# spawner1145/vae-tagger

Measured on AMD Instinct MI355X. Metric: images/sec encode+tag, 1024^2 bf16, higher is better.
Workload: dtype bf16

## Files before the change

### vae_tagger_amd/csrc/attn_qk.hip

```cpp
#include <hip/hip_runtime.h>

#include <type_traits>

#include "vt_common.h"
#include "vt_kernels.h"

namespace {

constexpr int QB = 256;
constexpr int KT = 64;
constexpr int D = 512;
constexpr int KROWB = D * 2;
constexpr int KBUF = KT * KROWB;

template <int MODE>
__global__ __launch_bounds__(512, 2) void attn_qk_kernel(const AttnQkArgs a) {
    extern __shared__ __attribute__((aligned(16))) char smem[];
    if (a.gate && *a.gate != a.gate_expect) return;
    const int lane = threadIdx.x & 63;
    const int wave = __builtin_amdgcn_readfirstlane(threadIdx.x >> 6);
    const int fr = lane & 15, fq = lane >> 4;
    const int qtiles = (a.S + QB - 1) / QB;
    const int nsplit = a.nsplit > 1 ? a.nsplit : 1;
    const int logical = vt_xcd_remap(blockIdx.x, gridDim.x);
    const int per_img = qtiles * nsplit;
    const int b = logical / per_img, qs = logical - b * per_img;
    const int qt = qs / nsplit, ksp = qs - qt * nsplit;
    const bf16_t* qb = a.q + (long long)b * a.qk_bs;
    constexpr bool LIN = MODE == 4 || MODE == 5;
    const bf16_t* kb = a.k + (long long)b * (LIN ? a.k_bs : a.qk_bs);
    const int nkeys = LIN ? a.nk : a.S;
    const int ldk = LIN ? a.ldk : a.ldq;
    const int row0 = qt * QB + wave * 32;

    bf16x8 qf[2][16];
#pragma unroll
    for (int j = 0; j < 2; ++j) {
        const int row = row0 + j * 16 + fr;
        const bf16_t* src = row < a.S ? qb + (long long)row * a.ldq + fq * 8 : (const bf16_t*)a.zeros;
        const int step = row < a.S ? 32 : 0;
#pragma unroll
        for (int ks = 0; ks < 16; ++ks) qf[j][ks] = *(const bf16x8*)(src + ks * step);
    }
    float rv[2];
    float sh2[2];
#pragma unroll
    for (int j = 0; j < 2; ++j) {
        const int row = row0 + j * 16 + fr;
        rv[j] = MODE == 1 ? -__builtin_inff() : 0.f;
        if (LIN) sh2[j] = (a.qbias && row < a.S) ? a.qbias[row] : 0.f;
        else sh2[j] = (MODE >= 2 && row < a.S) ? a.rowin[(long long)b * a.row_bs + row] * 1.44269504f : 0.f;
    }
    const float alpha2 = a.alpha * 1.44269504f;

    auto stage = [&](int kt, int buf) __attribute__((always_inline)) {
#pragma unroll
        for (int jj = 0; jj < 8; ++jj) {
            const int R = wave * 8 + jj;
            const int key = kt * KT + 32 * ((R >> 5) & 1) + 8 * ((R >> 2) & 3) + 4 * ((R >> 4) & 1) + (R & 3);
            const void* src = key < nkeys ? (const void*)(kb + (long long)key * ldk + ((lane ^ (R & 15)) << 3)) : a.zeros;
            __builtin_amdgcn_global_load_lds(VT_GLOBAL_PTR(src), VT_LDS_PTR(smem + buf * KBUF + R * KROWB), 16, 0, 0);
        }
    };
    int kbase[4];
#pragma unroll
    for (int m = 0; m < 4; ++m) kbase[m] = fr * KROWB + (((((m ^ (fr >> 2)) & 3) << 2) | ((fq ^ fr) & 3)) << 4);

    f32x4 acc[4][2];
    const f32x4 zero4 = {0.f, 0.f, 0.f, 0.f};

    bf16x8 hold[2][2];
    const int sr = lane >> 2, sp = lane & 3;
    const int perm_addr = (sp * 16 + sr) << 2;
    auto store_held = [&](int kt_prev) __attribute__((always_inline)) {
        if constexpr (MODE == 5) return;
        if constexpr (MODE == 3) {
            if (row0 < a.S) {
                bf16_t* dst = a.P + (long long)b * a.p_bs + (long long)(row0 >> 5) * vt_attn_pt_slab_stride(a.S) + (long long)kt_prev * 2048 + lane * 8;
#pragma unroll
                for (int j = 0; j < 2; ++j)
#pragma unroll
#ifdef PFRAG_PLAIN
                    for (int h = 0; h < 2; ++h) *(bf16x8*)(dst + (j * 2 + h) * 512) = hold[j][h];
#else
                    for (int h = 0; h < 2; ++h) __builtin_nontemporal_store(hold[j][h], (bf16x8*)(dst + (j * 2 + h) * 512));
#endif
            }
            return;
        }
        const int key0 = kt_prev * KT + 8 * sp;
        const bool full = kt_prev * KT + KT <= nkeys;
        if constexpr (MODE == 4) {
#pragma unroll
            for (int j = 0; j < 2; ++j) {
                const int row = row0 + j * 16 + sr;
                if (row < a.S) {
                    bf16_t* dst = a.P + (long long)b * a.p_bs + (long long)row * a.ldp + key0;
                    if (full || key0 < a.ldp) *(bf16x8*)dst = hold[j][0];
                    if (full || key0 + 32 < a.ldp) *(bf16x8*)(dst + 32) = hold[j][1];
                }
            }
            return;
        }
#pragma unroll
        for (int j = 0; j < 2; ++j) {
            const int row = row0 + j * 16 + sr;
            if (row < a.S) {
                bf16_t* dst = a.P + (long long)b * a.p_bs + (long long)row * a.ldp + key0;
                if (full || key0 < a.ldp) __builtin_nontemporal_store(hold[j][0], (bf16x8*)dst);
                if (full || key0 + 32 < a.ldp) __builtin_nontemporal_store(hold[j][1], (bf16x8*)(dst + 32));
            }
        }
    };
    auto epilogue_t = [&](int kt, auto full_tag) __attribute__((always_inline)) {
        constexpr bool FULL = decltype(full_tag)::value;
        const int key0 = kt * KT + 8 * fq;
        if constexpr (MODE == 5) {
            typedef _Float16 f16x8 __attribute__((ext_vector_type(8)));
            const int nrows = a.S - row0 < 0 ? 0 : (a.S - row0 > 32 ? 32 : a.S - row0);
            const long long ob = (long long)b * a.p_bs;
#pragma unroll
            for (int h = 0; h < 2; ++h) {
                const int kk = key0 + 32 * h;
                const bool kreal = FULL || kk + 7 < nkeys;
                f32x4 b0 = {0.f, 0.f, 0.f, 0.f}, b1 = b0;
                if (a.kbias && kreal) { b0 = *(const f32x4*)(a.kbias + kk); b1 = *(const f32x4*)(a.kbias + kk + 4); }
                float v[2][8];
#pragma unroll
                for (int j = 0; j < 2; ++j) {
                    const int row = row0 + j * 16 + fr;
                    const bool ok = row < a.S && kreal;
                    const long long o = ob + (long long)row * a.ldp + kk;
                    float rs[8] = {0.f, 0.f, 0.f, 0.f, 0.f, 0.f, 0.f, 0.f};
                    if (ok && a.res_f16) {
                        const f16x8 rh = *(const f16x8*)(a.res_f16 + o);
#pragma unroll
                        for (int e = 0; e < 8; ++e) rs[e] = (float)rh[e];
                    } else if (ok && a.res_f32) {
                        const f32x4 r0 = *(const f32x4*)(a.res_f32 + o), r1 = *(const f32x4*)(a.res_f32 + o + 4);
#pragma unroll
                        for (int e = 0; e < 4; ++e) { rs[e] = r0[e]; rs[4 + e] = r1[e]; }
                    }
#pragma unroll
                    for (int e = 0; e < 8; ++e)
                        v[j][e] = fmaf(acc[2 * h + (e >> 2)][j][e & 3], a.alpha, (e < 4 ? b0[e & 3] : b1[e & 3]) + sh2[j]) + rs[e];
                    if (ok && a.out_f16) {
                        f16x8 oh;
#pragma unroll
                        for (int e = 0; e < 8; ++e) oh[e] = (f16_t)v[j][e];
                        *(f16x8*)(a.out_f16 + o) = oh;
                    } else if (ok && a.out_f32) {
                        *(f32x4*)(a.out_f32 + o) = f32x4{v[j][0], v[j][1], v[j][2], v[j][3]};
                        *(f32x4*)(a.out_f32 + o + 4) = f32x4{v[j][4], v[j][5], v[j][6], v[j][7]};
                    }
                }
                if (a.gn_partial && kreal) {
                    const float piv = __shfl(v[0][0], lane & 32, 64);
                    float s1 = 0.f, s2 = 0.f;
#pragma unroll
                    for (int j = 0; j < 2; ++j) {
                        if (row0 + j * 16 + fr < a.S) {
#pragma unroll
                            for (int e = 0; e < 8; ++e) { const float d = v[j][e] - piv; s1 += d; s2 = fmaf(d, d, s2); }
                        }
                    }
                    s1 = vt_row16_sum(s1); s2 = vt_row16_sum(s2);
                    s1 += __shfl_xor(s1, 16, 64); s2 += __shfl_xor(s2, 16, 64);
                    if (fr == 0 && (fq & 1) == 0) {
                        const float n = (float)nrows * 16.f;
                        const float ms = n > 0.f ? s1 / n : 0.f;
                        float* d = a.gn_partial + (((long long)b * a.gn_parts + (row0 >> 5)) * (nkeys >> 4) + (kk >> 4)) * 3;
                        d[0] = n; d[1] = n > 0.f ? piv + ms : 0.f; d[2] = n > 0.f ? fmaxf(s2 - s1 * ms, 0.f) : 0.f;
                    }
                }
            }
            return;
        }
#pragma unroll
        for (int j = 0; j < 2; ++j) {
#pragma unroll
            for (int i = 0; i < 4; ++i)
#pragma unroll
                for (int r = 0; r < 4; ++r) {
                    const bool real = FULL || key0 + 32 * (i >> 1) + 4 * (i & 1) + r < nkeys;
                    if (MODE == 1) {
                        if (real) rv[j] = fmaxf(rv[j], acc[i][j][r] * a.alpha);
                    } else if (MODE == 4) {
                        const int kk = key0 + 32 * (i >> 1) + 4 * (i & 1) + r;
                        const float kbv = (a.kbias && real) ? a.kbias[kk] : 0.f;
                        hold[j][i >> 1][(i & 1) * 4 + r] = (bf16_t)(real ? fmaf(acc[i][j][r], a.alpha, kbv + sh2[j]) : 0.f);
                    } else {
                        float e = __builtin_amdgcn_exp2f(fmaf(acc[i][j][r], alpha2, -sh2[j]));
                        if (!real) e = 0.f;
                        rv[j] += e;
                        hold[j][i >> 1][(i & 1) * 4 + r] = (bf16_t)e;
                    }
                }
        }
        if (MODE == 2 || MODE == 4) {
            typedef int i32x4 __attribute__((ext_vector_type(4)));
#pragma unroll
            for (int j = 0; j < 2; ++j)
#pragma unroll
                for (int h = 0; h < 2; ++h) {
                    i32x4 v = __builtin_bit_cast(i32x4, hold[j][h]);
#pragma unroll
                    for (int d = 0; d < 4; ++d) v[d] = __builtin_amdgcn_ds_bpermute(perm_addr, v[d]);
                    hold[j][h] = __builtin_bit_cast(bf16x8, v);
                }
        }
    };
    const int nkt_all = (nkeys + KT - 1) / KT;
    const int segb[5] = {0, nkt_all / 4, nkt_all / 2, (int)(3LL * nkt_all / 4), nkt_all};
    auto write_segment = [&](int seg, bool zero) __attribute__((always_inline)) {
#pragma unroll
        for (int j = 0; j < 2; ++j) {
            float v = zero ? 0.f : rv[j];
            v += __shfl_xor(v, 16);
            v += __shfl_xor(v, 32);
            const int row = row0 + j * 16 + fr;
            if (fq == 0 && row < a.S) a.rowout[(long long)seg * a.split_stride + (long long)b * a.row_bs + row] = v;
            rv[j] = 0.f;
        }
    };
    auto epilogue = [&](int kt) __attribute__((always_inline)) {
        if (kt * KT + KT <= nkeys) epilogue_t(kt, std::true_type{});
        else epilogue_t(kt, std::false_type{});
        if (MODE == 3) {
#pragma unroll
            for (int seg = 0; seg < 4; ++seg)
                if (kt + 1 == segb[seg + 1] && segb[seg + 1] > segb[seg]) write_segment(seg, false);
        }
    };

    const bool late = (wave & 4) != 0;
    const int seg0 = ksp * (4 / nsplit), seg1 = (ksp + 1) * (4 / nsplit);
    const int kt0 = MODE == 3 ? segb[seg0] : LIN ? (int)((long long)ksp * nkt_all / nsplit) : 0;
    const int nkt = MODE == 3 ? segb[seg1] : LIN ? (int)((long long)(ksp + 1) * nkt_all / nsplit) : nkt_all;
    const bool counted = MODE == 3 && row0 < a.S;
    stage(kt0, kt0 & 1);
    for (int kt = kt0; kt < nkt; ++kt) {
        if (counted && kt - kt0 > (late ? 1 : 0)) asm volatile("s_waitcnt vmcnt(4)" ::: "memory");
        else asm volatile("s_waitcnt vmcnt(0)" ::: "memory");
        __builtin_amdgcn_s_barrier();
        asm volatile("" ::: "memory");
        if (late) {
            if (kt + 1 < nkt) stage(kt + 1, (kt + 1) & 1);
            if (kt > kt0) { epilogue(kt - 1); if (MODE >= 2) store_held(kt - 1); }
        }
        const char* ks_base = smem + (kt & 1) * KBUF;
        constexpr int AHEAD = 6;
        bf16x8 kf[8];
        auto frag = [&](int idx) __attribute__((always_inline)) {
            const int ks = idx >> 2, i = idx & 3;
            return *(const bf16x8*)(ks_base + kbase[ks & 3] + (ks >> 2) * 256 + i * 16 * KROWB);
        };
#pragma unroll
        for (int p = 0; p < AHEAD; ++p) kf[p] = frag(p);
#pragma unroll
        for (int idx = 0; idx < 64; ++idx) {
            if (idx + AHEAD < 64) kf[(idx + AHEAD) & 7] = frag(idx + AHEAD);
            const int ks = idx >> 2, i = idx & 3;
#pragma unroll
            for (int j = 0; j < 2; ++j)
                acc[i][j] = __builtin_amdgcn_mfma_f32_16x16x32_bf16(kf[idx & 7], qf[j][ks], ks == 0 ? zero4 : acc[i][j], 0, 0, 0);
            __builtin_amdgcn_sched_barrier(0);
        }
        if (!late) {
            if (kt + 1 < nkt) stage(kt + 1, (kt + 1) & 1);
            epilogue(kt);
            if (MODE >= 2) store_held(kt);
        }
    }
    if (nkt > kt0 && late) {
        epilogue(nkt - 1);
        if (MODE >= 2) store_held(nkt - 1);
    }
    if constexpr (LIN) return;
    if (MODE == 3) {
#pragma unroll
        for (int seg = 0; seg < 4; ++seg)
            if (seg >= seg0 && seg < seg1 && segb[seg + 1] == segb[seg]) write_segment(seg, true);
        return;
    }
#pragma unroll
    for (int j = 0; j < 2; ++j) {
        float v = rv[j];
        const float o1 = __shfl_xor(v, 16);
        v = MODE == 1 ? fmaxf(v, o1) : v + o1;
        const float o2 = __shfl_xor(v, 32);
        v = MODE == 1 ? fmaxf(v, o2) : v + o2;
        const int row = row0 + j * 16 + fr;
        if (fq == 0 && row < a.S) a.rowout[(long long)b * a.row_bs + row] = MODE == 1 ? v : 1.f / v;
    }
}

}

bool vt_attn_qk_supported(int S, int C) { return C == D && S > 0; }

int vt_attn_linear_parts(int S) { return (S + QB - 1) / QB * 8; }

hipError_t vt_launch_attn_qk(const AttnQkArgs& a, hipStream_t s) {
    if (a.mode == 5) {
        if (!a.q || !a.k || !a.zeros || a.batch <= 0 || !vt_attn_qk_supported(a.S, a.C) || a.nk <= 0 || (a.nk % 16) || a.gate) return hipErrorInvalidValue;
        if ((a.out_f16 != nullptr) == (a.out_f32 != nullptr) || (a.res_f16 && a.res_f32)) return hipErrorInvalidValue;
        if ((a.ldq % 8) || (a.ldk % 8) || (a.qk_bs % 8) || (a.k_bs % 8) || (a.ldp % 8) || (a.p_bs % 8) || a.ldp < a.nk) return hipErrorInvalidValue;
        if ((long long)a.S * a.ldq >= (1LL << 31) || (long long)a.nk * a.ldk >= (1LL << 31)) return hipErrorInvalidValue;
        if (a.gn_partial && a.gn_parts != vt_attn_linear_parts(a.S)) return hipErrorInvalidValue;
        const int nsp = a.nsplit > 1 ? a.nsplit : 1;
        if (nsp > (a.nk + KT - 1) / KT) return hipErrorInvalidValue;
        const long long nblk5 = (long long)((a.S + QB - 1) / QB) * a.batch * nsp;
        if (nblk5 > 0x7fffffffLL) return hipErrorInvalidValue;
        static std::atomic<unsigned long long> attr5{0};
        hipError_t e5 = vt_once_per_device(attr5, [&] { return hipFuncSetAttribute((const void*)attn_qk_kernel<5>, hipFuncAttributeMaxDynamicSharedMemorySize, 2 * KBUF); });
        if (e5 != hipSuccess) return e5;
        hipLaunchKernelGGL(attn_qk_kernel<5>, dim3((unsigned)nblk5), dim3(512), 2 * KBUF, s, a);
        return hipGetLastError();
    }
    if (a.mode == 4) {
        if (!a.q || !a.k || !a.P || !a.zeros || a.batch <= 0 || !vt_attn_qk_supported(a.S, a.C) || a.nk <= 0 || a.gate) return hipErrorInvalidValue;
        if ((a.ldq % 8) || (a.ldk % 8) || (a.qk_bs % 8) || (a.k_bs % 8) || (a.ldp % 8) || (a.p_bs % 8) || a.ldp < (a.nk + 7) / 8 * 8) return hipErrorInvalidValue;
        if ((long long)a.S * a.ldq >= (1LL << 31) || (long long)a.nk * a.ldk >= (1LL << 31)) return hipErrorInvalidValue;
        const int nsp = a.nsplit > 1 ? a.nsplit : 1;
        if (nsp > (a.nk + KT - 1) / KT) return hipErrorInvalidValue;
        const long long nblk4 = (long long)((a.S + QB - 1) / QB) * a.batch * nsp;
        if (nblk4 > 0x7fffffffLL) return hipErrorInvalidValue;
        static std::atomic<unsigned long long> attr4{0};
        hipError_t e4 = vt_once_per_device(attr4, [&] { return hipFuncSetAttribute((const void*)attn_qk_kernel<4>, hipFuncAttributeMaxDynamicSharedMemorySize, 2 * KBUF); });
        if (e4 != hipSuccess) return e4;
        hipLaunchKernelGGL(attn_qk_kernel<4>, dim3((unsigned)nblk4), dim3(512), 2 * KBUF, s, a);
        return hipGetLastError();
    }
    if (!a.q || !a.k || !a.rowout || !a.zeros || a.batch <= 0 || !vt_attn_qk_supported(a.S, a.C)) return hipErrorInvalidValue;
    if (a.mode != 1 && a.mode != 2) return hipErrorInvalidValue;
    if (a.mode == 2 && (!a.P || !a.rowin || (a.p_bs % 8))) return hipErrorInvalidValue;
    if (a.mode == 2 && !a.p_frag && ((a.ldp % 8) || a.ldp < a.S)) return hipErrorInvalidValue;
    if (a.mode == 2 && a.p_frag && a.p_bs < vt_attn_pt_elems(a.S)) return hipErrorInvalidValue;
    if ((a.ldq % 8) || (a.qk_bs % 8) || a.row_bs < a.S) return hipErrorInvalidValue;
    if ((long long)a.S * a.ldq >= (1LL << 31)) return hipErrorInvalidValue;
    if (a.nsplit > 1 && (a.mode != 2 || !a.p_frag || (a.nsplit != 2 && a.nsplit != 4))) return hipErrorInvalidValue;
    if (a.mode == 2 && a.p_frag && a.split_stride < (long long)a.batch * a.row_bs) return hipErrorInvalidValue;
    const long long nblk = (long long)((a.S + QB - 1) / QB) * a.batch * (a.nsplit > 1 ? a.nsplit : 1);
    if (nblk > 0x7fffffffLL) return hipErrorInvalidValue;
    static std::atomic<unsigned long long> attr_done{0};
    hipError_t ea = vt_once_per_device(attr_done, [&] {
        hipError_t e = hipFuncSetAttribute((const void*)attn_qk_kernel<1>, hipFuncAttributeMaxDynamicSharedMemorySize, 2 * KBUF);
        if (e == hipSuccess) e = hipFuncSetAttribute((const void*)attn_qk_kernel<2>, hipFuncAttributeMaxDynamicSharedMemorySize, 2 * KBUF);
        if (e == hipSuccess) e = hipFuncSetAttribute((const void*)attn_qk_kernel<3>, hipFuncAttributeMaxDynamicSharedMemorySize, 2 * KBUF);
        return e;
    });
    if (ea != hipSuccess) return ea;
    if (a.mode == 1) hipLaunchKernelGGL(attn_qk_kernel<1>, dim3((unsigned)nblk), dim3(512), 2 * KBUF, s, a);
    else if (a.p_frag) hipLaunchKernelGGL(attn_qk_kernel<3>, dim3((unsigned)nblk), dim3(512), 2 * KBUF, s, a);
    else hipLaunchKernelGGL(attn_qk_kernel<2>, dim3((unsigned)nblk), dim3(512), 2 * KBUF, s, a);
    return hipGetLastError();
}
```

### vae_tagger_amd/csrc/conv3x3_halo.hip

```cpp
#include <type_traits>

#include "vt_common.h"
#include "vt_kernels.h"

#ifdef GNIL_DUMP
extern "C" int vt_debug_gnil_dump(float* buf) { return (int)hipMemcpyToSymbol(HIP_SYMBOL(g_gnil_dump), &buf, sizeof(buf)); }
#endif
#ifdef HALO_STAMP
__device__ unsigned long long* g_halo_stamps = nullptr;
extern "C" int vt_debug_halo_stamps(unsigned long long* buf) {
    return (int)hipMemcpyToSymbol(HIP_SYMBOL(g_halo_stamps), &buf, sizeof(buf));
}
static unsigned long long* s_stamp_ptrs[2] = {nullptr, nullptr};
static int s_stamp_H = 0, s_stamp_Cin = 0, s_stamp_nth = -1, s_stamp_seen = 0;
static bool s_stamp_on = false;
extern "C" int vt_debug_halo_stamps_nth(unsigned long long* buf, int H, int Cin, int nth) {
    s_stamp_ptrs[1] = buf; s_stamp_H = H; s_stamp_Cin = Cin; s_stamp_nth = buf ? nth : -1; s_stamp_seen = 0; s_stamp_on = false;
    return (int)hipMemcpyToSymbol(HIP_SYMBOL(g_halo_stamps), &s_stamp_ptrs[0], sizeof(void*));
}
#ifndef STAMP_TID
#define STAMP_TID 0
#endif
#define STAMP(slot)                                                                                            \
    do {                                                                                                       \
        unsigned long long t_;                                                                                 \
        __builtin_amdgcn_sched_barrier(0);                                                                     \
        asm volatile("s_memrealtime %0\n\ts_waitcnt lgkmcnt(0)" : "=s"(t_)::"memory");                         \
        __builtin_amdgcn_sched_barrier(0);                                                                     \
        if (g_halo_stamps && threadIdx.x == STAMP_TID) g_halo_stamps[(long long)blockIdx.x * 16 + (slot)] = t_; \
    } while (0)
#define STAMP_CLK(slot)                                                                                        \
    do {                                                                                                       \
        unsigned long long t_;                                                                                 \
        __builtin_amdgcn_sched_barrier(0);                                                                     \
        asm volatile("s_memtime %0\n\ts_waitcnt lgkmcnt(0)" : "=s"(t_)::"memory");                             \
        __builtin_amdgcn_sched_barrier(0);                                                                     \
        if (g_halo_stamps && threadIdx.x == STAMP_TID) g_halo_stamps[(long long)blockIdx.x * 16 + (slot)] = t_; \
    } while (0)
#else
#define STAMP(slot) do {} while (0)
#define STAMP_CLK(slot) do {} while (0)
#endif

namespace {

template <bool F16>
__device__ __forceinline__ f32x4 halo_mfma(bf16x8 a, bf16x8 b, f32x4 c) {
#ifdef HALO_F16
    constexpr bool H = true;
#else
    constexpr bool H = F16;
#endif
#ifdef GNIL_NO_MFMA
    asm volatile("" :: "v"(a), "v"(b));
    return c;
#endif
    if constexpr (H) {
        typedef _Float16 f16x8 __attribute__((ext_vector_type(8)));
        return __builtin_amdgcn_mfma_f32_16x16x32_f16(__builtin_bit_cast(f16x8, a), __builtin_bit_cast(f16x8, b), c, 0, 0, 0);
    } else {
        return __builtin_amdgcn_mfma_f32_16x16x32_bf16(a, b, c, 0, 0, 0);
    }
}

constexpr int HB = 64;
constexpr int TW = 16;
constexpr int HWID = TW + 2;
constexpr int NW_DEFAULT = 6;

__device__ __forceinline__ void wait_vmcnt(int n) {
    switch (n) {
#define C(k) case k: asm volatile("s_waitcnt vmcnt(" #k ")" ::: "memory"); break;
        C(0) C(1) C(2) C(3) C(4) C(5) C(6) C(7) C(8) C(9) C(10) C(11) C(12) C(13) C(14) C(15) C(16)
        C(17) C(18) C(19) C(20) C(21) C(22) C(23) C(24)
#undef C
        default: asm volatile("s_waitcnt vmcnt(0)" ::: "memory"); break;
    }
}

template <typename V>
__device__ __forceinline__ void wait_vmcnt_tied(int n, V& r0, V& r1) {
    switch (n) {
#define C(k) case k: asm volatile("s_waitcnt vmcnt(" #k ")" : "+v"(r0), "+v"(r1)::"memory"); break;
        C(0) C(1) C(2) C(3) C(4) C(5) C(6) C(7) C(8) C(9) C(10) C(11) C(12) C(13) C(14) C(15) C(16)
#undef C
        default: asm volatile("s_waitcnt vmcnt(0)" : "+v"(r0), "+v"(r1)::"memory"); break;
    }
}


__device__ __forceinline__ int opaque(int v) {
    asm volatile("" : "+v"(v));
    return v;
}

template <typename V>
__device__ __forceinline__ void wait_vmcnt_tied1(int n, V& r0) {
    switch (n) {
#define C(k) case k: asm volatile("s_waitcnt vmcnt(" #k ")" : "+v"(r0)::"memory"); break;
        C(0) C(1) C(2) C(3) C(4) C(5) C(6) C(7) C(8) C(9) C(10) C(11) C(12) C(13) C(14) C(15) C(16)
#undef C
        default: asm volatile("s_waitcnt vmcnt(0)" : "+v"(r0)::"memory"); break;
    }
}

template <int WP, int WC, int XT, int TPW, int NW, bool F16 = false>
__global__ __launch_bounds__(64 * WP * WC, TPW == 4 ? 4 : TPW == 16 ? 1 : 2)
void conv3x3_halo_kernel(const Conv3x3Args a) {
    static_assert(!F16 || XT == 0, "fp16 operands: plain-input tiles only");
    constexpr int NWV = WP * WC;
    constexpr int NT = 64 * NWV;
    static_assert((NWV == 8 && (TPW == 8 || (TPW == 4 && XT == 0))) || (NWV == 4 && (TPW == 8 || TPW == 16) && XT == 0),
                  "8 waves x 8 rows, 8 waves x 4 rows (two workgroups per CU), 4 waves x 8 rows (two workgroups per CU), or -- the round-4 "
                  "experiment -- 4 waves x 16 rows: ONE wave per SIMD with up to 512 registers (accumulators in AGPRs)");
    constexpr int ROWS = WP * TPW;
    constexpr int BC = WC * 64;
    constexpr int TP = TPW, TC = 4;
    constexpr int HROWS = (ROWS + 2) * HWID;
    constexpr int NLD = NWV;
    constexpr int NXW = ((HROWS + 15) / 16 + NLD - 1) / NLD;
    constexpr int XBUF = NXW * NLD * 16 * HB;
    constexpr int WPCS = BC / 16;
    constexpr int WPW = (WPCS + NLD - 1) / NLD;
    constexpr int WBUF = BC * HB;
    constexpr int LX = XT == 1 ? 2 : 1;
    constexpr int DLY = XT == 1 ? 2 : 3;
    static_assert(WPW >= 1, "BC >= 128");
    static_assert(XT == 0 || NXW + DLY <= 9, "staging must finish inside the chunk");

    extern __shared__ __attribute__((aligned(16))) char smem[];
    char* const xbase = smem;
    char* const wbase = smem + 2 * XBUF;
    float* const ssl = (float*)(wbase + NW * WBUF);

    const int lane = threadIdx.x & 63;
    const int wave = __builtin_amdgcn_readfirstlane(threadIdx.x >> 6);
    const int wp = wave / WC, wc = wave % WC;
    const bool early = wave < 4;
    const int wpw = (WPCS % NLD == 0) ? WPW : (wave < WPCS % NLD ? WPW : WPW - 1);

    STAMP(0);
    const int tiles_x = a.tiles_x, ctiles = a.ctiles, per_img = a.per_img;
    auto fdiv = [](int n, unsigned long long m, int d) -> int {
        return m ? (int)(((unsigned long long)(unsigned)n * m) >> 40) : n / d;
    };
    int logical = vt_xcd_remap(blockIdx.x, gridDim.x);
    const int b = fdiv(logical, a.m_per_img, per_img);
    logical -= b * per_img;
    const int tile = fdiv(logical, a.m_ctiles, ctiles);
    const int ct = logical - tile * ctiles;
    const int tyi = fdiv(tile, a.m_tiles_x, tiles_x);
    const int ty0 = tyi * ROWS, tx0 = (tile - tyi * tiles_x) * TW;
    const int c0 = ct * BC;

    const long long img = (long long)b * a.H * a.W * a.Cin;
    const bf16_t* Xb = a.X ? a.X + img : nullptr;
    const float* Xf = a.Xf32 ? a.Xf32 + img : nullptr;
    const int nchunk = a.Cin >> 5;
    const int nk = nchunk * 9;

    const int drow = lane >> 2;
    const int dchunk = (lane & 3) ^ (((lane >> 4) & 1) << 1);
    constexpr int NXS = XT == 0 ? 1 : NXW;
    int xsrc[NXS];
    if constexpr (XT != 0) {
#pragma unroll
        for (int j = 0; j < NXW; ++j) {
            const int hr = (j * NLD + wave) * 16 + drow;
            const int hy = hr / HWID, hx = hr - hy * HWID;
            const int iy = ty0 - 1 + hy, ix = tx0 - 1 + hx;
            const bool v = hr < HROWS && iy >= 0 && iy < a.H && ix >= 0 && ix < a.W;
            xsrc[j] = v ? (iy * a.W + ix) * a.Cin + dchunk * 8 : -1;
        }
    } else {
        xsrc[0] = 0;
    }
    const int hr0 = wave * 16 + drow;
    const int hy0 = hr0 / HWID, hx0 = hr0 - (hr0 / HWID) * HWID;
    const int wsrc0 = (c0 + wave * 16 + drow) * 32 + dchunk * 8;
    const int wstep = a.Cout * 32;

    auto issue_x_dma = [&](int chunk) {
#ifdef EXP_NO_DMA
        if (chunk >= 2) return;
#endif
        char* dst = xbase + (chunk & 1) * XBUF;
        int hy = opaque(hy0), hx = hx0, hr = hr0;
#pragma nounroll
        for (int j = 0; j < NXW; ++j) {
            const int iy = ty0 - 1 + hy, ix = tx0 - 1 + hx;
            const bool v = hr < HROWS && iy >= 0 && iy < a.H && ix >= 0 && ix < a.W;
            const void* src = v ? (const void*)(Xb + ((iy * a.W + ix) * a.Cin + dchunk * 8 + chunk * 32)) : a.zeros;
#ifndef GNIL_NO_DMA
            __builtin_amdgcn_global_load_lds(VT_GLOBAL_PTR(src), VT_LDS_PTR(dst + (j * NLD + wave) * 1024), 16, 0, 0);
#else
            asm volatile("" :: "v"(src));
#endif
            hr += NLD * 16;
            hx += (NLD * 16) % HWID; hy += (NLD * 16) / HWID;
            if (hx >= HWID) { hx -= HWID; ++hy; }
        }
    };
    constexpr bool KYMAJOR = XT == 0 && TPW == 4;
    auto issue_w = [&](int t, int tap_of_t ) {
#ifdef EXP_NO_DMA
        if (t >= NW) return;
#endif
        char* dst = wbase + (t % NW) * WBUF;
        const int src_t = KYMAJOR ? t - tap_of_t + vt_halo_step_of_tap(tap_of_t) : t;
#ifdef W_WINDOW_EXPERIMENT
        const bf16_t* wt = a.Wp + (long long)(src_t % W_WINDOW_EXPERIMENT) * wstep + opaque(wsrc0);
#else
        const bf16_t* wt = a.Wp + (long long)src_t * wstep + opaque(wsrc0);
#endif
#pragma unroll
        for (int j = 0; j < WPW; ++j)
            if (WPCS % NLD == 0 || j * NLD + wave < WPCS)
#ifndef GNIL_NO_DMA
                __builtin_amdgcn_global_load_lds(VT_GLOBAL_PTR(wt + j * NLD * 16 * 32), VT_LDS_PTR(dst + (j * NLD + wave) * 1024), 16, 0, 0);
#else
                asm volatile("" :: "v"(wt));
#endif
    };
    auto load_row = [&](int j, int chunk, f32x4& r0, f32x4& r1) {
        const int xs_j = opaque(xsrc[j]);
        const int off = xs_j >= 0 ? xs_j + chunk * 32 : 0;
        if constexpr (XT == 1) {
            const float* src = xs_j >= 0 ? Xf + off : (const float*)a.zeros;
            asm volatile("global_load_dwordx4 %0, %1, off" : "=v"(r0) : "v"(src) : "memory");
            asm volatile("global_load_dwordx4 %0, %1, off offset:16" : "=v"(r1) : "v"(src) : "memory");
        } else {
            const bf16_t* src = xs_j >= 0 ? Xb + off : (const bf16_t*)a.zeros;
            asm volatile("global_load_dwordx4 %0, %1, off" : "=v"(r0) : "v"(src) : "memory");
        }
    };
    auto write_row = [&](int j, int chunk, const f32x4& r0, const f32x4& r1) {
        const float* sp = ssl + (chunk * 32 + opaque(dchunk) * 8) * 2;
        char* dst = xbase + (chunk & 1) * XBUF + (j * NLD + wave) * 1024 + opaque(lane) * 16;
        const bool pad = xsrc[j] < 0;
#pragma unroll
        for (int hh = 0; hh < 2; ++hh) {
            float v[4];
            if constexpr (XT == 1) {
                const f32x4 r = hh ? r1 : r0;
                v[0] = r[0]; v[1] = r[1]; v[2] = r[2]; v[3] = r[3];
            } else {
                const bf16x8 h = __builtin_bit_cast(bf16x8, r0);
#pragma unroll
                for (int i = 0; i < 4; ++i) v[i] = (float)h[hh * 4 + i];
            }
            const f32x4 q0 = *(const f32x4*)(sp + hh * 8), q1 = *(const f32x4*)(sp + hh * 8 + 4);
            bf16x4 o;
            o[0] = (bf16_t)vt_silu(fmaf(v[0], q0[0], q0[1]));
            o[1] = (bf16_t)vt_silu(fmaf(v[1], q0[2], q0[3]));
            o[2] = (bf16_t)vt_silu(fmaf(v[2], q1[0], q1[1]));
            o[3] = (bf16_t)vt_silu(fmaf(v[3], q1[2], q1[3]));
            if (pad) o = bf16x4{0, 0, 0, 0};
            *(bf16x4*)(dst + hh * 8) = o;
        }
    };

    constexpr bool SPF = XT == 0;
    constexpr int LEAD = NW - 1;
    constexpr int WOUT = SPF ? LEAD - 2 : NW - 2;
    const int fr = lane & 15, fq = lane >> 4;
    f32x4 bv[4];
#pragma unroll
    for (int i = 0; i < 4; ++i)
        bv[i] = a.bias ? *(const f32x4*)(a.bias + c0 + wc * 64 + 16 * fq + 4 * i) : f32x4{0.f, 0.f, 0.f, 0.f};
    asm volatile("" ::: "memory");
    if constexpr (XT == 0) {
        issue_x_dma(0);
#pragma unroll
        for (int t = 0; t < LEAD; ++t)
            if (t < nk) issue_w(t, t % 9);
        asm volatile("" ::: "memory");
    }
    const int wfoff = (wc * 64 + fr) * HB + ((fq ^ (((fr >> 2) & 1) << 1)) << 4);
    int xsel[8];
#pragma unroll
    for (int k = 0; k < 8; ++k)
        xsel[k] = (wp * TPW * HWID + fr) * HB + ((fq ^ ((((k + fr) >> 2) & 1) << 1)) << 4);
    auto xaddr = [&](int k) -> int { return xsel[k]; };
    f32x4 acc[TC][TP];
#pragma unroll
    for (int i = 0; i < TC; ++i) {
#pragma unroll
        for (int j = 0; j < TP; ++j) acc[i][j] = bv[i];
    }

    if constexpr (XT != 0) {
        const float* ssg = a.scale_shift + (long long)b * a.Cin * 2;
        for (int i = threadIdx.x; i < a.Cin * 2; i += NT) ssl[i] = ssg[i];
        __syncthreads();
#pragma unroll
        for (int j = 0; j < NXW; ++j) {
            f32x4 r0 = {0.f, 0.f, 0.f, 0.f}, r1 = {0.f, 0.f, 0.f, 0.f};
            load_row(j, 0, r0, r1);
            if constexpr (XT == 1) wait_vmcnt_tied(0, r0, r1);
            else wait_vmcnt_tied1(0, r0);
            write_row(j, 0, r0, r1);
        }
#pragma unroll
        for (int t = 0; t < LEAD; ++t)
            if (t < nk) issue_w(t, t % 9);
    }

    constexpr bool DYR = TPW >= 8;
    bf16x8 wfc[TC], xr[DYR ? TP + 2 : TP];
    STAMP(1);
    if constexpr (SPF) {
        int ahead0 = nk - 1;
        if (ahead0 > LEAD - 1) ahead0 = LEAD - 1;
        wait_vmcnt(ahead0 * wpw);
        asm volatile("" ::: "memory");
        __builtin_amdgcn_s_barrier();
        asm volatile("" ::: "memory");
        const char* ws0 = wbase + opaque(wfoff);
#pragma unroll
        for (int i = 0; i < TC; ++i) wfc[i] = *(const bf16x8*)(ws0 + i * 16 * HB);
#pragma unroll
        for (int r = 0; r < (DYR ? TP + 2 : TP); ++r) {
            const int rel = r * HWID;
            xr[r] = *(const bf16x8*)(xbase + xaddr(rel & 7) + rel * HB);
        }
    }
    STAMP(2);
    STAMP_CLK(11);

    auto do_chunk = [&](int chunk, auto last_tag) {
        constexpr bool LAST = decltype(last_tag)::value;
        const char* xs = xbase + (chunk & 1) * XBUF;
        const int tbase = chunk * 9;
        f32x4 rq[DLY][XT == 1 ? 2 : 1];
#pragma unroll
        for (int tap = 0; tap < 9; ++tap) {
            const int t = tbase + tap;
            if constexpr (!LAST) {
                int n = WOUT * wpw;
                if (XT == 0) { if (tap >= 1 && tap <= LEAD - 1) n += NXW; }
                else { for (int r = tap - (NW - 1); r <= tap - 1; ++r) if (r >= 0 && r < NXW) n += LX; }
                wait_vmcnt(n);
            } else {
                int ahead = 8 - tap - (SPF ? 1 : 0);
                if (ahead > WOUT) ahead = WOUT;
                if (ahead < 0) ahead = 0;
                wait_vmcnt(ahead * wpw);
            }
            if (XT != 0) asm volatile("s_waitcnt lgkmcnt(0)" ::: "memory");
            asm volatile("" ::: "memory");
            __builtin_amdgcn_s_barrier();
            asm volatile("" ::: "memory");
            if constexpr (!SPF) {
                if (!LAST || tap + LEAD < 9) issue_w(t + LEAD, (tap + LEAD) % 9);
            }

            if constexpr (SPF && !DYR) {
                const bool has_next = !LAST || tap < 8;
                const int tap_n = (tap + 1) % 9;
                const int dy_n = tap_n / 3, dx_n = tap_n % 3;
                const char* xs_n = (tap == 8) ? xbase + ((chunk + 1) & 1) * XBUF : xs;
                const char* ws_n = wbase + ((t + 1) % NW) * WBUF + opaque(wfoff);
                __builtin_amdgcn_s_setprio(1);
#pragma unroll
                for (int j = 0; j < TP; ++j) {
#pragma unroll
                    for (int i = 0; i < TC; ++i)
                        acc[i][j] = halo_mfma<F16>(wfc[i], xr[j], acc[i][j]);
                    if (has_next) {
                        const int rel = (j + dy_n) * HWID + dx_n;
                        xr[j] = *(const bf16x8*)(xs_n + xaddr(rel & 7) + rel * HB);
                    }
                    if (j == TP / 2 - 1) {
                        if (!LAST || tap + LEAD < 9) issue_w(t + LEAD, (tap + LEAD) % 9);
                        if constexpr (!LAST) { if (tap == 0) issue_x_dma(chunk + 1); }
                    }
                }
                __builtin_amdgcn_s_setprio(0);
                if (has_next) {
#pragma unroll
                    for (int i = 0; i < TC; ++i) wfc[i] = *(const bf16x8*)(ws_n + i * 16 * HB);
                }
                continue;
            }
            if constexpr (SPF) {
                const int dx = tap / 3, dy = tap % 3;
                const bool has_next = !LAST || tap < 8;
                const bool next_group = !LAST || dx < 2;
                const int dx_n = (dx + 1) % 3;
                const char* xs_n = (dx == 2) ? xbase + ((chunk + 1) & 1) * XBUF : xs;
                const char* ws_n = wbase + ((t + 1) % NW) * WBUF + opaque(wfoff);
                auto refill = [&](int r) {
#ifndef EXP_NO_FRAG_READS
                    const int rel = r * HWID + dx_n;
                    xr[r] = *(const bf16x8*)(xs_n + xaddr(rel & 7) + rel * HB);
#endif
                };
                __builtin_amdgcn_s_setprio(1);
#pragma unroll
                for (int j = 0; j < TP; ++j) {
#pragma unroll
                    for (int i = 0; i < TC; ++i)
                        acc[i][j] = halo_mfma<F16>(wfc[i], xr[j + dy], acc[i][j]);
                    if (next_group) {
                        if (dy == 0 && j == 0) refill(0);
                        if (dy == 1 && j == 0) refill(1);
                        if (dy == 2) refill(j + 2);
                    }
                    if (j == TP / 2 - 1) {
                        if (!LAST || tap + LEAD < 9) issue_w(t + LEAD, (tap + LEAD) % 9);
                        if constexpr (!LAST) { if (tap == 0) issue_x_dma(chunk + 1); }
                    }
                }
                __builtin_amdgcn_s_setprio(0);
#ifndef EXP_NO_FRAG_READS
                if (has_next) {
#pragma unroll
                    for (int i = 0; i < TC; ++i) wfc[i] = *(const bf16x8*)(ws_n + i * 16 * HB);
                }
#endif
                continue;
            }
            const char* ws = wbase + (t % NW) * WBUF + opaque(wfoff);
            const int dx = tap / 3, dy = tap % 3;
            bf16x8 wf[TC];
#pragma unroll
            for (int i = 0; i < TC; ++i) wf[i] = *(const bf16x8*)(ws + i * 16 * HB);

            constexpr bool STAGE = !LAST && XT != 0;
            const int r = tap - DLY;
            auto stage_row = [&]() {
                int n = DLY * wpw;
                for (int q = r + 1; q < tap; ++q) if (q < NXW) n += LX;
                if constexpr (XT == 1) wait_vmcnt_tied(n, rq[r % DLY][0], rq[r % DLY][1]);
                else wait_vmcnt_tied1(n, rq[r % DLY][0]);
                write_row(r, chunk + 1, rq[r % DLY][0], rq[r % DLY][XT == 1 ? 1 : 0]);
            };
            if constexpr (STAGE) {
                if (r >= 0 && r < NXW) {
                    if (early) stage_row();
                    __builtin_amdgcn_sched_barrier(0);
                }
            }
            __builtin_amdgcn_s_setprio(1);
#pragma unroll
            for (int jh = 0; jh < TP; jh += 4) {
                bf16x8 xf[4];
#pragma unroll
                for (int j = 0; j < 4; ++j) {
                    const int rel = (jh + j + dy) * HWID + dx;
                    xf[j] = *(const bf16x8*)(xs + xaddr(rel & 7) + rel * HB);
                }
#pragma unroll
                for (int j = 0; j < 4; ++j)
#pragma unroll
                    for (int i = 0; i < TC; ++i)
                        acc[i][jh + j] = halo_mfma<F16>(wf[i], xf[j], acc[i][jh + j]);
            }
            __builtin_amdgcn_s_setprio(0);
            if constexpr (STAGE) {
                if (r >= 0 && r < NXW) {
                    __builtin_amdgcn_sched_barrier(0);
                    if (!early) stage_row();
                }
                if (tap < NXW) load_row(tap, chunk + 1, rq[tap % DLY][0], rq[tap % DLY][XT == 1 ? 1 : 0]);
            }
        }
    };
    for (int chunk = 0; chunk + 1 < nchunk; ++chunk) do_chunk(chunk, std::false_type{});
    do_chunk(nchunk - 1, std::true_type{});
    if constexpr (XT == 0 && TPW >= 8) {
        if (a.scX) {
            const bf16_t* Xs = a.scX + (long long)b * a.H * a.W * a.scCin;
            const int scn = a.scCin >> 5;
#pragma nounroll
            for (int c = 0; c < scn; ++c) {
                asm volatile("s_waitcnt lgkmcnt(0)" ::: "memory");
                __builtin_amdgcn_s_barrier();
                asm volatile("" ::: "memory");
                {
                    int hy = opaque(hy0), hx = hx0, hr = hr0;
#pragma nounroll
                    for (int j = 0; j < NXW; ++j) {
                        const int iy = ty0 - 1 + hy, ix = tx0 - 1 + hx;
                        const bool v = hr < HROWS && iy >= 0 && iy < a.H && ix >= 0 && ix < a.W;
                        const void* src = v ? (const void*)(Xs + ((iy * a.W + ix) * a.scCin + dchunk * 8 + c * 32)) : a.zeros;
                        __builtin_amdgcn_global_load_lds(VT_GLOBAL_PTR(src), VT_LDS_PTR(xbase + (j * NLD + wave) * 1024), 16, 0, 0);
                        hr += NLD * 16;
                        hx += (NLD * 16) % HWID; hy += (NLD * 16) / HWID;
                        if (hx >= HWID) { hx -= HWID; ++hy; }
                    }
                    const bf16_t* wt = a.scW + (long long)c * wstep + opaque(wsrc0);
#pragma unroll
                    for (int j = 0; j < WPW; ++j)
                        if (WPCS % NLD == 0 || j * NLD + wave < WPCS)
                            __builtin_amdgcn_global_load_lds(VT_GLOBAL_PTR(wt + j * NLD * 16 * 32), VT_LDS_PTR(wbase + (j * NLD + wave) * 1024), 16, 0, 0);
                }
                wait_vmcnt(0);
                asm volatile("" ::: "memory");
                __builtin_amdgcn_s_barrier();
                asm volatile("" ::: "memory");
                const char* ws = wbase + opaque(wfoff);
                bf16x8 wf[TC];
#pragma unroll
                for (int i = 0; i < TC; ++i) wf[i] = *(const bf16x8*)(ws + i * 16 * HB);
#pragma unroll
                for (int jh = 0; jh < TP; jh += 4) {
                    bf16x8 xf[4];
#pragma unroll
                    for (int j = 0; j < 4; ++j) {
                        const int rel = (jh + j + 1) * HWID + 1;
                        xf[j] = *(const bf16x8*)(xbase + xaddr(rel & 7) + rel * HB);
                    }
#pragma unroll
                    for (int j = 0; j < 4; ++j)
#pragma unroll
                        for (int i = 0; i < TC; ++i)
                            acc[i][jh + j] = halo_mfma<F16>(wf[i], xf[j], acc[i][jh + j]);
                }
            }
        }
    }
    STAMP_CLK(12);
    STAMP(3);
#ifdef HALO_STAMP
    asm volatile("s_nop 0" :: "v"(acc[0][0]), "v"(acc[TC - 1][TP - 1]));
    STAMP(8);
#endif

    const int HWp = a.H * a.W;
    const long long ob = (long long)b * HWp * a.Cout;
    const int x = tx0 + fr;
    const int cw = c0 + wc * 64 + 16 * fq;
    constexpr int RPCS = TPW * 2;
    constexpr bool RES_DMA = NWV * RPCS * 1024 <= 2 * XBUF + NW * WBUF;
    char* const rbuf = smem + wave * (RPCS * 1024);
    if (RES_DMA && a.res_f16) {
        asm volatile("s_waitcnt lgkmcnt(0)" ::: "memory");
        __syncthreads();
#pragma unroll 4
        for (int pc = 0; pc < RPCS; ++pc) {
            const int pp = pc * 8 + (lane >> 3);
            const int yy = ty0 + wp * TPW + (pp >> 4), xx = tx0 + (pp & 15);
            const int lc = (lane & 7) ^ (pp & 7);
            const void* src = (yy < a.H && xx < a.W)
                ? (const void*)(a.res_f16 + ob + ((long long)yy * a.W + xx) * a.Cout + c0 + wc * 64 + lc * 8) : a.zeros;
            __builtin_amdgcn_global_load_lds(VT_GLOBAL_PTR(src), VT_LDS_PTR(rbuf + pc * 1024), 16, 0, 0);
        }
        asm volatile("s_waitcnt vmcnt(0)" ::: "memory");
    }
    unsigned valid = 0;
#pragma unroll
    for (int j = 0; j < TP; ++j) {
        const int y = ty0 + wp * TPW + j;
        if (y >= a.H || x >= a.W) continue;
        valid |= 1u << j;
        const long long o = ob + ((long long)y * a.W + x) * a.Cout + cw;
#pragma unroll
        for (int i = 0; i < TC; ++i) {
            f32x4 v = acc[i][j];
            if (a.res) v += *(const f32x4*)(a.res + o + 4 * i);
            if (a.out_f32) *(f32x4*)(a.out_f32 + o + 4 * i) = v;
            acc[i][j] = v;
        }
        if (a.res_f16) {
            const int pp = j * 16 + fr;
#pragma unroll
            for (int i = 0; i < TC; i += 2) {
                typedef _Float16 f16x8 __attribute__((ext_vector_type(8)));
                const f16x8 rh = RES_DMA ? *(const f16x8*)(rbuf + pp * 128 + (((2 * fq + (i >> 1)) ^ (pp & 7)) << 4))
                                         : *(const f16x8*)(a.res_f16 + o + 4 * i);
#pragma unroll
                for (int r = 0; r < 4; ++r) { acc[i][j][r] += (float)rh[r]; acc[i + 1][j][r] += (float)rh[4 + r]; }
            }
        }
        if (a.out_f16) {
#pragma unroll
            for (int i = 0; i < TC; i += 2) {
                typedef _Float16 f16x8 __attribute__((ext_vector_type(8)));
                f16x8 h;
#pragma unroll
                for (int r = 0; r < 4; ++r) { h[r] = (f16_t)acc[i][j][r]; h[4 + r] = (f16_t)acc[i + 1][j][r]; }
                *(f16x8*)(a.out_f16 + o + 4 * i) = h;
            }
        }
        if (a.out_bf16) {
            const long long o16 = a.out16_planar ? (((long long)(b * (a.Cout >> 5) + (cw >> 5)) * a.H + y) * a.W + x) * 32 + (cw & 31) : o;
#pragma unroll
            for (int i = 0; i < TC; i += 2) {
                if (a.out16_f16) {
                    typedef _Float16 f16x8o __attribute__((ext_vector_type(8)));
                    f16x8o h;
#pragma unroll
                    for (int r = 0; r < 4; ++r) { h[r] = (f16_t)acc[i][j][r]; h[4 + r] = (f16_t)acc[i + 1][j][r]; }
                    *(f16x8o*)((f16_t*)a.out_bf16 + o16 + 4 * i) = h;
                } else {
                bf16x8 h;
#pragma unroll
                for (int r = 0; r < 4; ++r) { h[r] = (bf16_t)acc[i][j][r]; h[4 + r] = (bf16_t)acc[i + 1][j][r]; }
#ifdef EPI_NOSTORE
                asm volatile("" :: "v"(h));
#else
                *(bf16x8*)(a.out_bf16 + o16 + 4 * i) = h;
#endif
                }
            }
        }
    }
    STAMP(4);
    if (a.gn_partial) {
        __syncthreads();
        STAMP(10);
        const int G = a.Cout / a.gn_cpg;
        float* out = a.gn_partial + (((long long)b * a.ptiles + tile) * G + c0 / a.gn_cpg) * 3;
        vt_gn_epilogue_partials_il<TC, TP>(acc, valid, a.gn_cpg, wp, WP, wc * 64, BC, (float*)smem, out);
    }
#ifdef HALO_STAMP
    STAMP(5);
    asm volatile("s_waitcnt vmcnt(0)" ::: "memory");
    STAMP(6);
    if (g_halo_stamps && threadIdx.x == STAMP_TID) {
        unsigned hw, xcc;
        asm volatile("s_getreg_b32 %0, hwreg(HW_REG_HW_ID)" : "=s"(hw));
        asm volatile("s_getreg_b32 %0, hwreg(HW_REG_XCC_ID)" : "=s"(xcc));
        g_halo_stamps[(long long)blockIdx.x * 16 + 7] = ((unsigned long long)xcc << 32) | hw;
    }
#endif
}

template <int WP, int WC, int XT, int TPW, int NW = NW_DEFAULT, bool F16 = false>
hipError_t launch(const Conv3x3Args& a, hipStream_t s) {
    constexpr int ROWS = WP * TPW, BC = WC * 64, NWV = WP * WC;
    constexpr int HROWS = (ROWS + 2) * HWID;
    constexpr int NXW = ((HROWS + 15) / 16 + NWV - 1) / NWV;
    const int smem = 2 * NXW * NWV * 16 * HB + NW * BC * HB + (XT ? a.Cin * 8 : 0);
    if (smem > 160 * 1024) return hipErrorInvalidValue;
    static std::atomic<unsigned long long> attr_done{0};
    auto kern = conv3x3_halo_kernel<WP, WC, XT, TPW, NW, F16>;
    hipError_t ea = vt_once_per_device(attr_done, [&] { return hipFuncSetAttribute((const void*)kern, hipFuncAttributeMaxDynamicSharedMemorySize, 160 * 1024); });
    if (ea != hipSuccess) return ea;
    const long long tiles = (long long)((a.W + TW - 1) / TW) * ((a.H + ROWS - 1) / ROWS);
    const long long nblk = tiles * (a.Cout / BC) * a.batch;
    if (nblk <= 0 || nblk > 0x7fffffffLL) return hipErrorInvalidValue;
    Conv3x3Args k = a;
    k.tiles_x = (a.W + TW - 1) / TW; k.ctiles = a.Cout / BC; k.per_img = (int)(tiles * k.ctiles); k.ptiles = (int)tiles;
    auto magic = [&](long long d) -> unsigned long long {
        return (nblk * d < (1LL << 40) && nblk < (1LL << 23)) ? ((1ULL << 40) / (unsigned long long)d + 1ULL) : 0ULL;
    };
    k.m_per_img = magic(k.per_img); k.m_ctiles = magic(k.ctiles); k.m_tiles_x = magic(k.tiles_x);
#ifdef HALO_STAMP
    if (s_stamp_nth >= 0) {
        const bool on = a.H == s_stamp_H && a.Cin == s_stamp_Cin && s_stamp_seen++ == s_stamp_nth;
        if (on != s_stamp_on) {
            (void)hipMemcpyToSymbolAsync(HIP_SYMBOL(g_halo_stamps), &s_stamp_ptrs[on ? 1 : 0], sizeof(void*), 0, hipMemcpyHostToDevice, s);
            s_stamp_on = on;
        }
    }
#endif
#ifdef GNIL_ONE_WG
    hipLaunchKernelGGL(kern, dim3((unsigned)nblk), dim3(64 * NWV), smem > 90 * 1024 ? smem : 90 * 1024, s, k);
#else
    hipLaunchKernelGGL(kern, dim3((unsigned)nblk), dim3(64 * NWV), smem, s, k);
#endif
    return hipGetLastError();
}

__global__ void repack_ohwi_kernel(const bf16_t* __restrict__ w, bf16_t* __restrict__ wp, int Cin, int Cout) {
    const long long n = (long long)Cout * 9 * Cin;
    const long long i = (long long)blockIdx.x * blockDim.x + threadIdx.x;
    if (i >= n) return;
    const int ci = (int)(i % Cin);
    const int tap = (int)((i / Cin) % 9);
    const int co = (int)(i / ((long long)Cin * 9));
    const int row = (co & ~63) + vt_halo_row_of_cout(co & 63);
    wp[(((long long)(ci >> 5) * 9 + vt_halo_step_of_tap(tap)) * Cout + row) * 32 + (ci & 31)] = w[i];
}

}

hipError_t vt_launch_repack_ohwi_to_halo(const bf16_t* w, bf16_t* wp, int Cin, int Cout, hipStream_t s) {
    const long long n = (long long)Cout * 9 * Cin;
    hipLaunchKernelGGL(repack_ohwi_kernel, dim3((unsigned)((n + 255) / 256)), dim3(256), 0, s, w, wp, Cin, Cout);
    return hipGetLastError();
}

namespace {
enum HaloVariant { HV_2208_4 = 0, HV_4204_4, HV_4208_6, HV_2408_6, HV_XT1_128, HV_XT1_256, HV_XT2_128, HV_XT2_256, HV_2216_6 };
HaloVariant halo_variant(int Cout, int xt, int occ2, bool has_sc) {
    const bool big = (Cout % 256) == 0;
    if (xt == 1) return big ? HV_XT1_256 : HV_XT1_128;
    if (xt == 2) return big ? HV_XT2_256 : HV_XT2_128;
    if (occ2 == 4) return HV_2216_6;
    if (occ2 == 3 || (occ2 == 2 && !big)) return HV_2208_4;
    if (occ2 && !big && !has_sc) return HV_4204_4;
    return big ? HV_2408_6 : HV_4208_6;
}
int halo_variant_rows(HaloVariant v) {
    switch (v) {
        case HV_4208_6: case HV_XT1_128: case HV_XT2_128: case HV_2216_6: return 32;
        default: return 16;
    }
}
}

int vt_conv3x3_halo_tiles(int H, int W, int Cout, int xt, int occ2, int has_sc) {
    const int rows = halo_variant_rows(halo_variant(Cout, xt, occ2, has_sc != 0));
    return ((W + TW - 1) / TW) * ((H + rows - 1) / rows);
}
int vt_conv3x3_halo_tiles_max(int H, int W) { return ((W + TW - 1) / TW) * ((H + 15) / 16); }

bool vt_conv3x3_halo_supported(int Cin, int Cout) { return Cin >= 32 && (Cin % 32) == 0 && (Cout % 128) == 0; }
bool vt_conv3x3_halo_f16_supported(int Cout, int occ2, int has_sc) { return halo_variant(Cout, 0, occ2, has_sc != 0) == HV_2208_4; }

static int halo_xt(const Conv3x3Args& a) { return a.scale_shift ? (a.Xf32 ? 1 : 2) : 0; }

int vt_conv3x3_halo_config(const Conv3x3Args& a) {
    switch (halo_variant(a.Cout, halo_xt(a), a.occ2, a.scX != nullptr)) {
        case HV_2208_4: return 3;
        case HV_4204_4: return 4;
        case HV_4208_6: return 5;
        case HV_2408_6: return 6;
        case HV_2216_6: return 5;
        case HV_XT1_128: case HV_XT1_256: return 7;
        default: return 8;
    }
}

hipError_t vt_launch_conv3x3_halo(const Conv3x3Args& a, hipStream_t s) {
    if (!a.Wp || !a.zeros || (!a.out_f32 && !a.out_bf16 && !a.out_f16)) return hipErrorInvalidValue;
    if ((a.res && a.res_f16) || (a.res_f16 && a.out_f32)) return hipErrorInvalidValue;
    if (!vt_conv3x3_halo_supported(a.Cin, a.Cout) || a.batch <= 0 || a.H <= 0 || a.W <= 0) return hipErrorInvalidValue;
    if (a.gn_partial && a.gn_cpg != 4 && a.gn_cpg != 8 && a.gn_cpg != 16) return hipErrorInvalidValue;
    if ((long long)a.H * a.W * a.Cin >= (1LL << 31)) return hipErrorInvalidValue;
    if ((a.scX != nullptr) != (a.scW != nullptr)) return hipErrorInvalidValue;
    if (a.scX && (a.scCin <= 0 || (a.scCin % 32) || a.scale_shift || (long long)a.H * a.W * a.scCin >= (1LL << 31))) return hipErrorInvalidValue;
    if ((long long)(a.Cin / 32) * 9 * a.Cout * 32 >= (1LL << 31)) return hipErrorInvalidValue;
    if (a.occ2 < 0 || a.occ2 > 4) return hipErrorInvalidValue;
    const int xt = halo_xt(a);
    if (xt == 1 ? (a.X != nullptr) : (a.X == nullptr || a.Xf32 != nullptr)) return hipErrorInvalidValue;
    if (a.f16 && (xt != 0 || halo_variant(a.Cout, xt, a.occ2, a.scX != nullptr) != HV_2208_4)) return hipErrorInvalidValue;
    if (a.f16) return launch<2, 2, 0, 8, 4, true>(a, s);
    switch (halo_variant(a.Cout, xt, a.occ2, a.scX != nullptr)) {
        case HV_2208_4: return launch<2, 2, 0, 8, 4>(a, s);
        case HV_4204_4: return launch<4, 2, 0, 4, 4>(a, s);
        case HV_4208_6: return launch<4, 2, 0, 8>(a, s);
        case HV_2408_6: return launch<2, 4, 0, 8>(a, s);
        case HV_2216_6: return launch<2, 2, 0, 16, 6>(a, s);
        case HV_XT1_128: return launch<4, 2, 1, 8>(a, s);
        case HV_XT1_256: return launch<2, 4, 1, 8>(a, s);
        case HV_XT2_128: return launch<4, 2, 2, 8>(a, s);
        default: return launch<2, 4, 2, 8>(a, s);
    }
}
```

### vae_tagger_amd/csrc/conv3x3_s2_halo.hip

```cpp
#include <type_traits>

#include "vt_common.h"
#include "vt_kernels.h"

namespace {

constexpr int HB = 64;
constexpr int TW = 16, ROWS = 16;
constexpr int WP = 2, WC = 2, TP = 8, TC = 4;
constexpr int NWV = WP * WC, NT = 64 * NWV, BC = WC * 64;
constexpr int NW = 3, LEAD = NW - 1;
constexpr int WBUF = BC * HB;
constexpr int WPW = BC / 16 / NWV;
constexpr int NXB = 3;
#ifndef S2_W_AT
#define S2_W_AT (TP / 2 - 1)
#endif
constexpr int XSTRIDE = 289 * HB;
constexpr int SMEM = NXB * XSTRIDE + NW * WBUF;
static_assert(2 * SMEM <= 160 * 1024, "two workgroups per CU");

__host__ __device__ constexpr int pl_py(int pl) { return pl >> 1; }
__host__ __device__ constexpr int pl_px(int pl) { return pl & 1; }
__host__ __device__ constexpr int pl_pitch(int pl) { return pl_px(pl) ? 16 : 17; }
__host__ __device__ constexpr int pl_hrows(int pl) { return pl_py(pl) ? 16 : 17; }
__host__ __device__ constexpr int pl_rows(int pl) { return pl_pitch(pl) * pl_hrows(pl); }
__host__ __device__ constexpr int pl_pieces(int pl) { return pl_rows(pl) / 16; }
__host__ __device__ constexpr int nx_pl(int pl) { return pl == 3 ? 4 : 5; }
__host__ __device__ constexpr int st_plane(int p) { return p < 4 ? 0 : p < 6 ? 1 : p < 8 ? 2 : 3; }
__host__ __device__ constexpr int st_dx(int p) { return (p == 2 || p == 3 || p == 7) ? 1 : 0; }
__host__ __device__ constexpr int st_dy(int p) { return (p == 1 || p == 3 || p == 5) ? 1 : 0; }
__host__ __device__ constexpr bool st_two(int p) { return p < 6; }
__host__ __device__ constexpr int ng_plane(int p) { return p < 2 ? 0 : p < 4 ? 1 : p < 7 ? 2 : p < 8 ? 3 : 0; }
__host__ __device__ constexpr int ng_dx(int p) { return (p < 2 || p == 6) ? 1 : 0; }
__host__ __device__ constexpr int ng_rows(int p) { return (p < 4 || p == 8) ? 9 : 8; }

__device__ __forceinline__ void wait_vmcnt(int n) {
    switch (n) {
#define C(k) case k: asm volatile("s_waitcnt vmcnt(" #k ")" ::: "memory"); break;
        C(0) C(1) C(2) C(3) C(4) C(5) C(6) C(7) C(8) C(9) C(10) C(11) C(12)
#undef C
        default: asm volatile("s_waitcnt vmcnt(0)" ::: "memory"); break;
    }
}
__device__ __forceinline__ int opaque(int v) {
    asm volatile("" : "+v"(v));
    return v;
}
__device__ __forceinline__ int opaque_s(int v) {
    asm volatile("" : "+s"(v));
    return v;
}

template <bool F16>
__global__ __launch_bounds__(NT, 2) void conv3x3_s2_halo_kernel(const Conv3x3S2Args a) {
    extern __shared__ __attribute__((aligned(16))) char smem[];
    char* const xbase = smem;
    char* const wbase = smem + NXB * XSTRIDE;
    const int lane = threadIdx.x & 63;
    const int wave = __builtin_amdgcn_readfirstlane(threadIdx.x >> 6);
    const int wp = wave / WC, wc = wave % WC;
    const int fr = lane & 15, fq = lane >> 4;

    auto fdiv = [](int n, unsigned long long m, int d) -> int {
        return m ? (int)(((unsigned long long)(unsigned)n * m) >> 40) : n / d;
    };
    int logical = vt_xcd_remap(blockIdx.x, gridDim.x);
    const int b = fdiv(logical, a.m_per_img, a.per_img);
    logical -= b * a.per_img;
    const int tile = fdiv(logical, a.m_ctiles, a.ctiles);
    const int ct = logical - tile * a.ctiles;
    const int tyi = fdiv(tile, a.m_tiles_x, a.tiles_x);
    const int ty0 = tyi * ROWS, tx0 = (tile - tyi * a.tiles_x) * TW;
    const int c0 = ct * BC;
    const bf16_t* Xb = a.X + (long long)b * a.H * a.W * a.Cin;
    const int xpix = a.x_planar ? 32 : a.Cin, xchunk = a.x_planar ? a.H * a.W * 32 : 32;
    const int nchunk = a.Cin >> 5;
    const int nk = nchunk * 9;

    const int drow = lane >> 2;
    const int dchunk = (lane & 3) ^ (((lane >> 4) & 1) << 1);
    const int wsrc0 = (c0 + wave * 16 + drow) * 32 + dchunk * 8;
    const int wstep = a.Cout * 32;

    auto issue_x = [&](auto pl_tag, int chunk, int slot) {
        constexpr int PL = decltype(pl_tag)::value;
        constexpr int PITCH = pl_pitch(PL), PY = pl_py(PL), PX = pl_px(PL), NP = pl_pieces(PL), NXP = nx_pl(PL);
        constexpr int NPT = PL == 0 ? NP + 1 : NP;
        char* dst = xbase + slot * XSTRIDE;
#pragma nounroll
        for (int j = 0; j < NXP; ++j) {
            int piece = j * NWV + wave;
            if (piece >= NPT) piece = NPT - 1;
            const int row0 = (PL == 0 && piece == NP) ? pl_rows(0) - 16 : piece * 16;
            const int hr = row0 + opaque(drow);
            const int hy = hr / PITCH, hx = hr - hy * PITCH;
            const int iy = 2 * (ty0 + hy) + PY, ix = 2 * (tx0 + hx) + PX;
            const int lch = (lane & 3) ^ (((hr >> 2) & 1) << 1);
            const void* src = (iy < a.H && ix < a.W) ? (const void*)(Xb + ((iy * a.W + ix) * xpix + chunk * xchunk + lch * 8)) : a.zeros;
            __builtin_amdgcn_global_load_lds(VT_GLOBAL_PTR(src), VT_LDS_PTR(dst + row0 * HB), 16, 0, 0);
        }
    };
    auto issue_w = [&](int t) {
        char* dst = wbase + (t % NW) * WBUF;
        const bf16_t* wt = a.Wp + (long long)t * wstep + opaque(wsrc0);
#pragma unroll
        for (int j = 0; j < WPW; ++j)
            __builtin_amdgcn_global_load_lds(VT_GLOBAL_PTR(wt + j * NWV * 16 * 32), VT_LDS_PTR(dst + (j * NWV + wave) * 1024), 16, 0, 0);
    };

    issue_x(std::integral_constant<int, 0>{}, 0, 0);
    issue_w(0);
    issue_w(1);
    issue_x(std::integral_constant<int, 1>{}, 0, 1);
    asm volatile("" ::: "memory");

    const int wfoff = (wc * 64 + fr) * HB + ((fq ^ (((fr >> 2) & 1) << 1)) << 4);
    int xsel[8];
#pragma unroll
    for (int k = 0; k < 8; ++k) xsel[k] = fr * HB + ((fq ^ ((((k + fr) >> 2) & 1) << 1)) << 4);
    const int wpoff17 = wp * TP * 17 * HB, wpoff16 = wp * TP * 16 * HB;
    auto xfrag = [&](const char* buf , int pitch , int r, int dx) -> bf16x8 {
        const int rel = r * pitch + dx;
        return *(const bf16x8*)(buf + xsel[rel & 7] + rel * HB);
    };
    auto xfrag_after = [&](const char* buf, int pitch, int r, int dx, const f32x4& after) -> bf16x8 {
        const int rel = r * pitch + dx;
        int off = xsel[rel & 7];
        asm volatile("" : "+v"(off) : "v"(after));
        return *(const bf16x8*)(buf + off + rel * HB);
    };

    f32x4 acc[TC][TP];
#pragma unroll
    for (int i = 0; i < TC; ++i)
#pragma unroll
        for (int j = 0; j < TP; ++j) acc[i][j] = f32x4{0.f, 0.f, 0.f, 0.f};

    bf16x8 wfc[TC], xr[TP + 1];
    {
        wait_vmcnt(WPW + nx_pl(1));
        asm volatile("" ::: "memory");
        __builtin_amdgcn_s_barrier();
        asm volatile("" ::: "memory");
        const char* ws0 = wbase + opaque(wfoff);
#pragma unroll
        for (int i = 0; i < TC; ++i) wfc[i] = *(const bf16x8*)(ws0 + i * 16 * HB);
#pragma unroll
        for (int r = 0; r < TP + 1; ++r) xr[r] = xfrag(xbase + opaque_s(wpoff17), 17, r, 0);
    }

    int cm = 0;
    auto slot_of = [&](int cmod, int pl) -> int { const int s = cmod + pl; return s >= 3 ? (s >= 6 ? s - 6 : s - 3) : s; };

    auto do_chunk = [&](int chunk, auto last_tag) {
        constexpr bool LAST = decltype(last_tag)::value;
        const int tbase = chunk * 9;
        const int cmn = cm == 2 ? 0 : cm + 1;
#pragma unroll
        for (int p = 0; p < 9; ++p) {
            const int t = tbase + p;
            {
                int n = 0;
                if (p == 1) n = nx_pl(2);
                if (p == 4) n = nx_pl(3);
                if (p == 6 && !LAST) n = nx_pl(0);
                if (p == 0) n = nx_pl(1);
                wait_vmcnt(n);
            }
            asm volatile("" ::: "memory");
            __builtin_amdgcn_s_barrier();
            asm volatile("" ::: "memory");
            constexpr int dummy = 0; (void)dummy;
            const int pl = st_plane(p), dy = st_dy(p);
            const bool two = st_two(p);
            const bool has_next = !LAST || p < 8;
            const int npl = ng_plane(p), ndx = ng_dx(p), nrows = ng_rows(p);
            const int npitch = pl_pitch(npl);
            const bool next_chunk = p == 8;
            const char* xs_n = xbase + opaque_s(slot_of(next_chunk ? cmn : cm, npl) * XSTRIDE + (npitch == 17 ? wpoff17 : wpoff16));
            const char* ws_n = wbase + ((t + 1) % NW) * WBUF + opaque(wfoff);
            (void)pl;
            auto refill = [&](int r, const f32x4& after) {
                if (has_next && r < nrows) xr[r] = xfrag_after(xs_n, npitch, r, ndx, after);
            };
            __builtin_amdgcn_s_setprio(1);
#pragma unroll
            for (int j = 0; j < TP; ++j) {
#pragma unroll
                for (int i = 0; i < TC; ++i)
                    if constexpr (F16) {
                        typedef _Float16 f16x8m __attribute__((ext_vector_type(8)));
                        acc[i][j] = __builtin_amdgcn_mfma_f32_16x16x32_f16(__builtin_bit_cast(f16x8m, wfc[i]), __builtin_bit_cast(f16x8m, xr[two ? j + dy : j]), acc[i][j], 0, 0, 0);
                    } else {
                        acc[i][j] = __builtin_amdgcn_mfma_f32_16x16x32_bf16(wfc[i], xr[two ? j + dy : j], acc[i][j], 0, 0, 0);
                    }
                if (two) {
                    if (dy == 0) { if (j == 0) refill(0, acc[TC - 1][j]); }
                    else refill(j + 1, acc[TC - 1][j]);
                } else {
                    refill(j, acc[TC - 1][j]);
                    if (j == TP - 1) refill(TP, acc[TC - 1][j]);
                }
                if (j == S2_W_AT) {
                    if (!LAST || p + LEAD < 9) issue_w(t + LEAD);
                }
                if (j == TP / 2 - 1) {
                    if (p == 0) issue_x(std::integral_constant<int, 2>{}, chunk, slot_of(cm, 2));
                    if (p == 3) issue_x(std::integral_constant<int, 3>{}, chunk, slot_of(cm, 3));
                    if constexpr (!LAST) {
                        if (p == 5) issue_x(std::integral_constant<int, 0>{}, chunk + 1, slot_of(cmn, 0));
                        if (p == 8) issue_x(std::integral_constant<int, 1>{}, chunk + 1, slot_of(cmn, 1));
                    }
                }
            }
            __builtin_amdgcn_s_setprio(0);
            if (has_next) {
#pragma unroll
                for (int i = 0; i < TC; ++i) wfc[i] = *(const bf16x8*)(ws_n + i * 16 * HB);
            }
            __builtin_amdgcn_sched_barrier(0);
        }
        cm = cmn;
    };
    for (int chunk = 0; chunk + 1 < nchunk; ++chunk) do_chunk(chunk, std::false_type{});
    do_chunk(nchunk - 1, std::true_type{});
    (void)nk;
#pragma unroll
    for (int i = 0; i < TC; ++i)
#pragma unroll
        for (int j = 0; j < TP; ++j) asm volatile("" : "+v"(acc[i][j]));
    asm volatile("" ::: "memory");

    const long long ob = (long long)b * a.Ho * a.Wo * a.Cout;
    const int x = tx0 + fr;
    const int cw = c0 + wc * 64 + 16 * fq;
    f32x4 bv[4];
#pragma unroll
    for (int i = 0; i < 4; ++i) bv[i] = a.bias ? *(const f32x4*)(a.bias + cw + 4 * i) : f32x4{0.f, 0.f, 0.f, 0.f};
    unsigned valid = 0;
#pragma unroll
    for (int j = 0; j < TP; ++j) {
        const int y = ty0 + wp * TP + j;
        if (y >= a.Ho || x >= a.Wo) continue;
        valid |= 1u << j;
        const long long o = ob + ((long long)y * a.Wo + x) * a.Cout + cw;
#pragma unroll
        for (int i = 0; i < TC; ++i) {
            f32x4 v = acc[i][j] + bv[i];
            if (a.res) v += *(const f32x4*)(a.res + o + 4 * i);
            if (a.out_f32) *(f32x4*)(a.out_f32 + o + 4 * i) = v;
            acc[i][j] = v;
        }
        typedef _Float16 f16x8 __attribute__((ext_vector_type(8)));
        if (a.out_f16) {
#pragma unroll
            for (int i = 0; i < TC; i += 2) {
                f16x8 h;
#pragma unroll
                for (int r = 0; r < 4; ++r) { h[r] = (f16_t)acc[i][j][r]; h[4 + r] = (f16_t)acc[i + 1][j][r]; }
                *(f16x8*)(a.out_f16 + o + 4 * i) = h;
            }
        }
        if (a.out_bf16) {
#pragma unroll
            for (int i = 0; i < TC; i += 2) {
                if (a.out16_f16) {
                    f16x8 h;
#pragma unroll
                    for (int r = 0; r < 4; ++r) { h[r] = (f16_t)acc[i][j][r]; h[4 + r] = (f16_t)acc[i + 1][j][r]; }
                    *(f16x8*)((f16_t*)a.out_bf16 + o + 4 * i) = h;
                } else {
                    bf16x8 h;
#pragma unroll
                    for (int r = 0; r < 4; ++r) { h[r] = (bf16_t)acc[i][j][r]; h[4 + r] = (bf16_t)acc[i + 1][j][r]; }
                    *(bf16x8*)(a.out_bf16 + o + 4 * i) = h;
                }
            }
        }
    }
    if (a.gn_partial) {
        asm volatile("s_waitcnt lgkmcnt(0)" ::: "memory");
        __syncthreads();
        const int G = a.Cout / a.gn_cpg;
        float* out = a.gn_partial + (((long long)b * a.ptiles + tile) * G + c0 / a.gn_cpg) * 3;
        vt_gn_epilogue_partials_il<TC, TP>(acc, valid, a.gn_cpg, wp, WP, wc * 64, BC, (float*)smem, out);
    }
}

__global__ void repack_ohwi_s2_kernel(const bf16_t* __restrict__ w, bf16_t* __restrict__ wp, int Cin, int Cout) {
    const long long n = (long long)Cout * 9 * Cin;
    const long long i = (long long)blockIdx.x * blockDim.x + threadIdx.x;
    if (i >= n) return;
    const int ci = (int)(i % Cin);
    const int tap = (int)((i / Cin) % 9);
    const int co = (int)(i / ((long long)Cin * 9));
    const int row = (co & ~63) + vt_halo_row_of_cout(co & 63);
    wp[(((long long)(ci >> 5) * 9 + vt_s2_step_of_tap(tap)) * Cout + row) * 32 + (ci & 31)] = w[i];
}

}

bool vt_conv3x3_s2_supported(int Cin, int Cout) { return Cin >= 32 && (Cin % 32) == 0 && (Cout % 128) == 0; }
int vt_conv3x3_s2_tiles(int Ho, int Wo) { return ((Wo + TW - 1) / TW) * ((Ho + ROWS - 1) / ROWS); }

hipError_t vt_launch_repack_ohwi_to_s2(const bf16_t* w, bf16_t* wp, int Cin, int Cout, hipStream_t s) {
    const long long n = (long long)Cout * 9 * Cin;
    hipLaunchKernelGGL(repack_ohwi_s2_kernel, dim3((unsigned)((n + 255) / 256)), dim3(256), 0, s, w, wp, Cin, Cout);
    return hipGetLastError();
}

hipError_t vt_launch_conv3x3_s2(const Conv3x3S2Args& a, hipStream_t s) {
    if (!a.X || !a.Wp || !a.zeros || (!a.out_f32 && !a.out_bf16 && !a.out_f16)) return hipErrorInvalidValue;
    if (!vt_conv3x3_s2_supported(a.Cin, a.Cout) || a.batch <= 0 || a.H < 2 || a.W < 2) return hipErrorInvalidValue;
    if (a.gn_partial && a.gn_cpg != 4 && a.gn_cpg != 8 && a.gn_cpg != 16) return hipErrorInvalidValue;
    if ((long long)a.H * a.W * a.Cin >= (1LL << 31)) return hipErrorInvalidValue;
    if ((long long)(a.Cin / 32) * 9 * a.Cout * 32 >= (1LL << 31)) return hipErrorInvalidValue;
    static std::atomic<unsigned long long> attr_done{0};
    hipError_t ea = vt_once_per_device(attr_done, [&] {
        hipError_t e = hipFuncSetAttribute((const void*)conv3x3_s2_halo_kernel<false>, hipFuncAttributeMaxDynamicSharedMemorySize, SMEM);
        if (e == hipSuccess) e = hipFuncSetAttribute((const void*)conv3x3_s2_halo_kernel<true>, hipFuncAttributeMaxDynamicSharedMemorySize, SMEM);
        return e;
    });
    if (ea != hipSuccess) return ea;
    Conv3x3S2Args k = a;
    k.Ho = a.H / 2; k.Wo = a.W / 2;
    const long long tiles = vt_conv3x3_s2_tiles(k.Ho, k.Wo);
    const long long nblk = tiles * (a.Cout / BC) * a.batch;
    if (nblk <= 0 || nblk > 0x7fffffffLL) return hipErrorInvalidValue;
    k.tiles_x = (k.Wo + TW - 1) / TW; k.ctiles = a.Cout / BC; k.per_img = (int)(tiles * k.ctiles); k.ptiles = (int)tiles;
    auto magic = [&](long long d) -> unsigned long long {
        return (nblk * d < (1LL << 40) && nblk < (1LL << 23)) ? ((1ULL << 40) / (unsigned long long)d + 1ULL) : 0ULL;
    };
    k.m_per_img = magic(k.per_img); k.m_ctiles = magic(k.ctiles); k.m_tiles_x = magic(k.tiles_x);
    if (a.f16) hipLaunchKernelGGL(conv3x3_s2_halo_kernel<true>, dim3((unsigned)nblk), dim3(NT), SMEM, s, k);
    else hipLaunchKernelGGL(conv3x3_s2_halo_kernel<false>, dim3((unsigned)nblk), dim3(NT), SMEM, s, k);
    return hipGetLastError();
}
```

### vae_tagger_amd/csrc/conv3x3_up2.hip

```cpp
#include "vt_common.h"
#include "vt_kernels.h"

namespace {

constexpr int HB = 64;
constexpr int TW = 16;
constexpr int HWID = TW + 2;
constexpr int ROWS = 8;
constexpr int NWV = 4;
constexpr int TPW = 2;
constexpr int BC = 64;
constexpr int TC = 4;
constexpr int HROWS = (ROWS + 2) * HWID;
constexpr int XPCS = (HROWS + 15) / 16;
constexpr int XBUF = XPCS * 16 * HB;
constexpr int WBLK = BC * HB;
constexpr int WPCS = 16 * BC / 16;
constexpr int SMEM = XBUF + 16 * WBLK;

template <bool F16>
__device__ __forceinline__ f32x4 up2_mfma(bf16x8 a, bf16x8 b, f32x4 c) {
    if constexpr (F16) {
        typedef _Float16 f16x8 __attribute__((ext_vector_type(8)));
        return __builtin_amdgcn_mfma_f32_16x16x32_f16(__builtin_bit_cast(f16x8, a), __builtin_bit_cast(f16x8, b), c, 0, 0, 0);
    } else {
        return __builtin_amdgcn_mfma_f32_16x16x32_bf16(a, b, c, 0, 0, 0);
    }
}

template <bool F16>
__global__ __launch_bounds__(64 * NWV, 2)
void conv3x3_up2_kernel(const ConvUp2Args a) {
    extern __shared__ __attribute__((aligned(16))) char smem[];
    char* const xbase = smem;
    char* const wbase = smem + XBUF;

    const int lane = threadIdx.x & 63;
    const int wave = __builtin_amdgcn_readfirstlane(threadIdx.x >> 6);
    const int fr = lane & 15, fq = lane >> 4;

    int logical = vt_xcd_remap(blockIdx.x, gridDim.x);
    const int per_img = a.ptiles * a.ctiles;
    const int b = logical / per_img;
    logical -= b * per_img;
    const int tile = logical / a.ctiles;
    const int ct = logical - tile * a.ctiles;
    const int tyi = tile / a.tiles_x;
    const int ty0 = tyi * ROWS, tx0 = (tile - tyi * a.tiles_x) * TW;
    const int c0 = ct * BC;

    const bf16_t* Xb = a.X + (long long)b * a.H * a.W * a.Cin;
    const int nchunk = a.Cin >> 5;

    const int drow = lane >> 2;
    const int dchunk = (lane & 3) ^ (((lane >> 4) & 1) << 1);
    auto stage = [&](int chunk) {
#pragma nounroll
        for (int pc = wave; pc < XPCS; pc += NWV) {
            const int hr = pc * 16 + drow;
            const int hy = hr / HWID, hx = hr - hy * HWID;
            const int iy = ty0 - 1 + hy, ix = tx0 - 1 + hx;
            const bool v = hr < HROWS && iy >= 0 && iy < a.H && ix >= 0 && ix < a.W;
            const void* src = v ? (const void*)(Xb + ((iy * a.W + ix) * a.Cin + dchunk * 8 + chunk * 32)) : a.zeros;
            __builtin_amdgcn_global_load_lds(VT_GLOBAL_PTR(src), VT_LDS_PTR(xbase + pc * 1024), 16, 0, 0);
        }
        const bf16_t* wsrc = a.Wp + ((long long)chunk * 16 * a.Cout + c0 + drow) * 32 + dchunk * 8;
#pragma nounroll
        for (int pc = wave; pc < WPCS; pc += NWV) {
            const int q = pc >> 2, part = pc & 3;
            __builtin_amdgcn_global_load_lds(VT_GLOBAL_PTR(wsrc + ((long long)q * a.Cout + part * 16) * 32), VT_LDS_PTR(wbase + pc * 1024), 16, 0, 0);
        }
    };

    f32x4 acc[TC][8];
#pragma unroll
    for (int i = 0; i < TC; ++i) {
        const f32x4 bv = a.bias ? *(const f32x4*)(a.bias + c0 + 16 * fq + 4 * i) : f32x4{0.f, 0.f, 0.f, 0.f};
#pragma unroll
        for (int j = 0; j < 8; ++j) acc[i][j] = bv;
    }

    const int wfoff = fr * HB + ((fq ^ (((fr >> 2) & 1) << 1)) << 4);

#pragma nounroll
    for (int chunk = 0; chunk < nchunk; ++chunk) {
        __syncthreads();
        stage(chunk);
        asm volatile("s_waitcnt vmcnt(0)" ::: "memory");
        __syncthreads();
        bf16x8 xf[4][3];
#pragma unroll
        for (int r = 0; r < 4; ++r) {
#pragma unroll
            for (int s = 0; s < 3; ++s) {
                const int row = (wave * TPW + r) * HWID + s + fr;
                xf[r][s] = *(const bf16x8*)(xbase + row * HB + ((fq ^ (((row >> 2) & 1) << 1)) << 4));
            }
        }
#pragma unroll
        for (int p = 0; p < 4; ++p) {
            const int pa = p >> 1, pb = p & 1;
#pragma unroll
            for (int t = 0; t < 4; ++t) {
                const int ry = t >> 1, rx = t & 1;
                const char* ws = wbase + (p * 4 + t) * WBLK + wfoff;
                bf16x8 wf[TC];
#pragma unroll
                for (int i = 0; i < TC; ++i) wf[i] = *(const bf16x8*)(ws + i * 16 * HB);
#pragma unroll
                for (int j = 0; j < TPW; ++j) {
#pragma unroll
                    for (int i = 0; i < TC; ++i)
                        acc[i][p * 2 + j] = up2_mfma<F16>(wf[i], xf[j + ry + pa][rx + pb], acc[i][p * 2 + j]);
                }
            }
        }
    }

    const int Ho = 2 * a.H, Wo = 2 * a.W;
    const long long ob = (long long)b * Ho * Wo * a.Cout;
    const int lx = tx0 + fr;
    const int cw = c0 + 16 * fq;
    unsigned valid = 0;
#pragma unroll
    for (int p = 0; p < 4; ++p) {
#pragma unroll
        for (int j = 0; j < TPW; ++j) {
            const int ly = ty0 + wave * TPW + j;
            if (ly >= a.H || lx >= a.W) continue;
            const int jj = p * 2 + j;
            valid |= 1u << jj;
            const long long o = ob + ((long long)(2 * ly + (p >> 1)) * Wo + (2 * lx + (p & 1))) * a.Cout + cw;
            if (a.out_f32) {
#pragma unroll
                for (int i = 0; i < TC; ++i) *(f32x4*)(a.out_f32 + o + 4 * i) = acc[i][jj];
            }
            typedef _Float16 f16x8 __attribute__((ext_vector_type(8)));
            if (a.out_f16) {
#pragma unroll
                for (int i = 0; i < TC; i += 2) {
                    f16x8 h;
#pragma unroll
                    for (int r = 0; r < 4; ++r) { h[r] = (f16_t)acc[i][jj][r]; h[4 + r] = (f16_t)acc[i + 1][jj][r]; }
                    *(f16x8*)(a.out_f16 + o + 4 * i) = h;
                }
            }
            if (a.out_16) {
#pragma unroll
                for (int i = 0; i < TC; i += 2) {
                    if (a.out16_f16) {
                        f16x8 h;
#pragma unroll
                        for (int r = 0; r < 4; ++r) { h[r] = (f16_t)acc[i][jj][r]; h[4 + r] = (f16_t)acc[i + 1][jj][r]; }
                        *(f16x8*)((f16_t*)a.out_16 + o + 4 * i) = h;
                    } else {
                        bf16x8 h;
#pragma unroll
                        for (int r = 0; r < 4; ++r) { h[r] = (bf16_t)acc[i][jj][r]; h[4 + r] = (bf16_t)acc[i + 1][jj][r]; }
                        *(bf16x8*)(a.out_16 + o + 4 * i) = h;
                    }
                }
            }
        }
    }
    if (a.gn_partial) {
        __syncthreads();
        const int G = a.Cout / a.gn_cpg;
        float* out = a.gn_partial + (((long long)b * a.ptiles + tile) * G + c0 / a.gn_cpg) * 3;
        vt_gn_epilogue_partials_il<TC, 8>(acc, valid, a.gn_cpg, wave, NWV, 0, BC, (float*)smem, out);
    }
}

template <bool F16>
hipError_t launch_up2(const ConvUp2Args& a, hipStream_t s) {
    static std::atomic<unsigned long long> attr_done{0};
    auto kern = conv3x3_up2_kernel<F16>;
    hipError_t ea = vt_once_per_device(attr_done, [&] { return hipFuncSetAttribute((const void*)kern, hipFuncAttributeMaxDynamicSharedMemorySize, SMEM); });
    if (ea != hipSuccess) return ea;
    ConvUp2Args k = a;
    k.tiles_x = (a.W + TW - 1) / TW;
    k.ptiles = k.tiles_x * ((a.H + ROWS - 1) / ROWS);
    k.ctiles = a.Cout / BC;
    const long long nblk = (long long)k.ptiles * k.ctiles * a.batch;
    if (nblk <= 0 || nblk > 0x7fffffffLL) return hipErrorInvalidValue;
    hipLaunchKernelGGL(kern, dim3((unsigned)nblk), dim3(64 * NWV), SMEM, s, k);
    return hipGetLastError();
}

__global__ void pack_up2_kernel(const float* __restrict__ w, bf16_t* __restrict__ wp_bf16, f16_t* __restrict__ wp_f16, int Cin, int Cout) {
    const long long n = (long long)Cout * Cin * 16;
    const long long idx = (long long)blockIdx.x * blockDim.x + threadIdx.x;
    if (idx >= n) return;
    const int q = (int)(idx & 15);
    const int ci = (int)((idx >> 4) % Cin);
    const int co = (int)((idx >> 4) / Cin);
    const int pa = q >> 3, pb = (q >> 2) & 1, ry = (q >> 1) & 1, rx = q & 1;
    const int ky0 = pa == 0 ? (ry == 0 ? 0 : 1) : (ry == 0 ? 0 : 2), ky1 = pa == 0 ? (ry == 0 ? 0 : 2) : (ry == 0 ? 1 : 2);
    const int kx0 = pb == 0 ? (rx == 0 ? 0 : 1) : (rx == 0 ? 0 : 2), kx1 = pb == 0 ? (rx == 0 ? 0 : 2) : (rx == 0 ? 1 : 2);
    const float* wt = w + ((long long)co * Cin + ci) * 9;
    float sum = 0.f;
    bool first = true;
    for (int ky = ky0; ky <= ky1; ++ky)
        for (int kx = kx0; kx <= kx1; ++kx) {
            const float v = wt[ky * 3 + kx];
            sum = first ? v : __fadd_rn(sum, v);
            first = false;
        }
    const int row = (co & ~63) + vt_halo_row_of_cout(co & 63);
    const long long d = (((long long)(ci >> 5) * 16 + q) * Cout + row) * 32 + (ci & 31);
    if (wp_bf16) wp_bf16[d] = (bf16_t)sum;
    if (wp_f16) wp_f16[d] = (f16_t)sum;
}

__global__ void pack_f32_oihw_kernel(const float* __restrict__ w, bf16_t* __restrict__ dst, int Cin, int Cout, int layout, int f16) {
    const long long n = (long long)Cout * Cin * 9;
    const long long idx = (long long)blockIdx.x * blockDim.x + threadIdx.x;
    if (idx >= n) return;
    const int tap = (int)(idx % 9);
    const int ci = (int)((idx / 9) % Cin);
    const int co = (int)(idx / ((long long)Cin * 9));
    const int row = (co & ~63) + vt_halo_row_of_cout(co & 63);
    const long long d = layout == 0 ? ((long long)co * 9 + tap) * Cin + ci
                                    : (((long long)(ci >> 5) * 9 + vt_halo_step_of_tap(tap)) * Cout + row) * 32 + (ci & 31);
    if (f16) ((f16_t*)dst)[d] = (f16_t)w[idx]; else dst[d] = (bf16_t)w[idx];
}

__global__ __launch_bounds__(256)
void upsample2x_nhwc16_kernel(const uint4* __restrict__ x, uint4* __restrict__ y, int H, int W, int C8, long long n) {
    const long long idx = (long long)blockIdx.x * blockDim.x + threadIdx.x;
    if (idx >= n) return;
    const int c = (int)(idx % C8);
    long long p = idx / C8;
    const int X = (int)(p % (2 * W)); p /= 2 * W;
    const int Y = (int)(p % (2 * H));
    const long long b = p / (2 * H);
    y[idx] = x[((b * H + (Y >> 1)) * W + (X >> 1)) * C8 + c];
}

}

bool vt_conv3x3_up2_supported(int Cin, int Cout) { return Cin >= 32 && (Cin % 32) == 0 && Cout >= BC && (Cout % BC) == 0; }
int vt_conv3x3_up2_tiles(int H, int W) { return ((W + TW - 1) / TW) * ((H + ROWS - 1) / ROWS); }

hipError_t vt_launch_conv3x3_up2(const ConvUp2Args& a, hipStream_t s) {
    if (!a.X || !a.Wp || !a.zeros || (!a.out_f32 && !a.out_f16 && !a.out_16)) return hipErrorInvalidValue;
    if (!vt_conv3x3_up2_supported(a.Cin, a.Cout) || a.batch <= 0 || a.H <= 0 || a.W <= 0) return hipErrorInvalidValue;
    if (a.gn_partial && a.gn_cpg != 4 && a.gn_cpg != 8 && a.gn_cpg != 16) return hipErrorInvalidValue;
    if ((long long)a.H * a.W * a.Cin >= (1LL << 31)) return hipErrorInvalidValue;
    if ((long long)a.H * 2 + 1 >= (1LL << 30) || (long long)a.W * 2 + 1 >= (1LL << 30)) return hipErrorInvalidValue;
    return a.f16 ? launch_up2<true>(a, s) : launch_up2<false>(a, s);
}

hipError_t vt_launch_pack_up2(const float* w_oihw, bf16_t* wp_bf16, f16_t* wp_f16, int Cin, int Cout, hipStream_t s) {
    const long long n = (long long)Cout * Cin * 16;
    if (!w_oihw || (!wp_bf16 && !wp_f16) || n <= 0 || (n + 255) / 256 > 0x7fffffffLL) return hipErrorInvalidValue;
    hipLaunchKernelGGL(pack_up2_kernel, dim3((unsigned)((n + 255) / 256)), dim3(256), 0, s, w_oihw, wp_bf16, wp_f16, Cin, Cout);
    return hipGetLastError();
}

hipError_t vt_launch_pack_f32_oihw(const float* w_oihw, bf16_t* dst, int Cin, int Cout, int layout, int f16, hipStream_t s) {
    const long long n = (long long)Cout * Cin * 9;
    if (!w_oihw || !dst || n <= 0 || (n + 255) / 256 > 0x7fffffffLL || (layout == 1 && (Cin % 32 || Cout % 64))) return hipErrorInvalidValue;
    hipLaunchKernelGGL(pack_f32_oihw_kernel, dim3((unsigned)((n + 255) / 256)), dim3(256), 0, s, w_oihw, dst, Cin, Cout, layout, f16);
    return hipGetLastError();
}

hipError_t vt_launch_upsample2x_nhwc16(const void* x, void* y, int B, int H, int W, int C, hipStream_t s) {
    if (!x || !y || B <= 0 || H <= 0 || W <= 0 || C <= 0 || (C % 8)) return hipErrorInvalidValue;
    const long long n = (long long)B * 2 * H * 2 * W * (C / 8);
    if ((n + 255) / 256 > 0x7fffffffLL) return hipErrorInvalidValue;
    hipLaunchKernelGGL(upsample2x_nhwc16_kernel, dim3((unsigned)((n + 255) / 256)), dim3(256), 0, s, (const uint4*)x, (uint4*)y, H, W, C / 8, n);
    return hipGetLastError();
}
```

### vae_tagger_amd/csrc/conv_gemm.hip

```cpp
#include "vt_common.h"
#include "vt_kernels.h"

namespace {

constexpr int ROWB = 128;

template <int BP, int BC, int WP, int WC, bool F8 = false, bool F16 = false>
__device__ __forceinline__ void conv_gemm_tile(const ConvGemmArgs& a, char* smem, int logical) {
    static_assert(!(F8 && F16), "one operand type");
    static_assert(WP * WC == 8, "8 waves per workgroup");
    constexpr int ES = F8 ? 1 : 2;
    constexpr int BK = ROWB / ES;
    constexpr int CE = 16 / ES;
    constexpr int TP = BP / WP / 16;
    constexpr int TC = BC / WC / 16;
    constexpr int XI = BP / 8;
    constexpr int WI = BC / 8;
    constexpr int NXJ = (XI + 7) / 8;
    constexpr int NWJ = (WI + 7) / 8;
    constexpr int STAGE_BYTES = (BP + BC) * ROWB;

    const int lane = threadIdx.x & 63;
    const int wave = __builtin_amdgcn_readfirstlane(threadIdx.x >> 6);
    const int wp = wave / WC, wc = wave % WC;

    const int HWo = a.Hout * a.Wout;
    const int ptiles = (HWo + BP - 1) / BP;
    const int ctiles = (a.Cout + BC - 1) / BC;
    const int per_img = ptiles * ctiles;
    const int b = logical / per_img;
    logical -= b * per_img;
    const int p0 = (logical / ctiles) * BP;
    const int c0 = (logical % ctiles) * BC;

    const char* Xb = (const char*)a.X + (long long)b * a.x_bs * ES;
    const char* Wb = (const char*)a.W + (long long)b * a.w_bs * ES;

    const int lrow = lane >> 3;
    const int lchunk = (lane & 7) ^ lrow;
    const int ntaps = a.ksize * a.ksize;
    const int ncb = (a.Cin + BK - 1) / BK;
    const bool chunk_tail_possible = (a.Cin % BK) != 0;

    int xoff[NXJ];
    unsigned xmask[NXJ];
#pragma unroll
    for (int j = 0; j < NXJ; ++j) {
        const int r = (j * 8 + wave) * 8 + lrow;
        const int p = p0 + r;
        const bool rv = (r < BP) && (p < HWo);
        const int oy = p / a.Wout, ox = p - oy * a.Wout;
        const int iy0 = oy * a.stride - a.pad, ix0 = ox * a.stride - a.pad;
        xoff[j] = (iy0 * a.Win + ix0) * a.ldx + lchunk * CE;
        unsigned m = 0;
        if (rv) {
            for (int t = 0; t < ntaps; ++t) {
                const int ky = t / a.ksize, kx = t - ky * a.ksize;
                const int iy = iy0 + ky, ix = ix0 + kx;
                if (iy >= 0 && iy < a.Hin && ix >= 0 && ix < a.Win) m |= 1u << t;
            }
        }
        xmask[j] = m;
    }
    int woff[NWJ];
    bool wvalid[NWJ];
#pragma unroll
    for (int j = 0; j < NWJ; ++j) {
        const int rblk = j * 8 + wave;
        const int rl = rblk * 8 + lrow;
        const int n = c0 + (TC == 4 ? (rl & ~63) + (rl & 3) + 4 * ((rl >> 4) & 3) + 16 * ((rl >> 2) & 3) : rl);
        wvalid[j] = (rblk < WI) && (n < a.Wrows);
        woff[j] = n * a.ldw + lchunk * CE;
    }

    auto stage = [&](int tap, int cb, int buf) {
        char* xs = smem + buf * STAGE_BYTES;
        char* ws = xs + BP * ROWB;
        const int ky = (tap * 11) >> 5, kx = tap - ky * 3;
        const int doff = (a.ksize == 1) ? 0 : (ky * a.Win + kx) * a.ldx;
        const int k0 = cb * BK;
        const bool cv = !chunk_tail_possible || (k0 + lchunk * CE < a.Cin);
#pragma unroll
        for (int j = 0; j < NXJ; ++j) {
            const int rblk = j * 8 + wave;
            if (XI % 8 == 0 || rblk < XI) {
                const bool v = ((xmask[j] >> tap) & 1u) && cv;
                const void* src = v ? (const void*)(Xb + (long long)(xoff[j] + doff + k0) * ES) : a.zeros;
                if (a.x_stream) __builtin_amdgcn_global_load_lds(VT_GLOBAL_PTR(src), VT_LDS_PTR(xs + rblk * 1024), 16, 0, 2);
                else __builtin_amdgcn_global_load_lds(VT_GLOBAL_PTR(src), VT_LDS_PTR(xs + rblk * 1024), 16, 0, 0);
            }
        }
#pragma unroll
        for (int j = 0; j < NWJ; ++j) {
            const int rblk = j * 8 + wave;
            if (WI % 8 == 0 || rblk < WI) {
                const bool v = wvalid[j] && cv;
                const void* src = v ? (const void*)(Wb + (long long)(woff[j] + tap * a.Cin + k0) * ES) : a.zeros;
                __builtin_amdgcn_global_load_lds(VT_GLOBAL_PTR(src), VT_LDS_PTR(ws + rblk * 1024), 16, 0, 0);
            }
        }
    };

    const int frow = lane & 15;
    const int fq = lane >> 4;
    const int foff0 = frow * ROWB + (((0 + fq) ^ (lane & 7)) << 4);
    const int foff1 = frow * ROWB + (((4 + fq) ^ (lane & 7)) << 4);

    f32x4 acc[TC][TP];
#pragma unroll
    for (int i = 0; i < TC; ++i)
#pragma unroll
        for (int j = 0; j < TP; ++j) acc[i][j] = f32x4{0.f, 0.f, 0.f, 0.f};

    const int nk = ntaps * ncb;
    stage(0, 0, 0);
    int tap_n = 0, cb_n = 1;
    if (cb_n == ncb) { cb_n = 0; tap_n = 1; }

    for (int t = 0; t < nk; ++t) {
        __syncthreads();
        if (t + 1 < nk) {
            stage(tap_n, cb_n, (t + 1) & 1);
            if (++cb_n == ncb) { cb_n = 0; ++tap_n; }
        }
        const char* xs = smem + (t & 1) * STAGE_BYTES + (wp * (BP / WP)) * ROWB;
        const char* ws = smem + (t & 1) * STAGE_BYTES + BP * ROWB + (wc * (BC / WC)) * ROWB;
        if constexpr (F8) {
            typedef int i32x4 __attribute__((ext_vector_type(4)));
            typedef int i32x8 __attribute__((ext_vector_type(8)));
            const int fa = frow * ROWB + (((2 * fq) ^ (lane & 7)) << 4), fb = frow * ROWB + (((2 * fq + 1) ^ (lane & 7)) << 4);
            i32x8 wf[TC], xf[TP];
#pragma unroll
            for (int i = 0; i < TC; ++i) {
                const i32x4 lo = *(const i32x4*)(ws + i * 16 * ROWB + fa), hi = *(const i32x4*)(ws + i * 16 * ROWB + fb);
                wf[i] = i32x8{lo[0], lo[1], lo[2], lo[3], hi[0], hi[1], hi[2], hi[3]};
            }
#pragma unroll
            for (int j = 0; j < TP; ++j) {
                const i32x4 lo = *(const i32x4*)(xs + j * 16 * ROWB + fa), hi = *(const i32x4*)(xs + j * 16 * ROWB + fb);
                xf[j] = i32x8{lo[0], lo[1], lo[2], lo[3], hi[0], hi[1], hi[2], hi[3]};
            }
#pragma unroll
            for (int i = 0; i < TC; ++i)
#pragma unroll
                for (int j = 0; j < TP; ++j)
                    acc[i][j] = __builtin_amdgcn_mfma_scale_f32_16x16x128_f8f6f4(wf[i], xf[j], acc[i][j], 0, 0, 0, 127, 0, 127);
        } else {
#pragma unroll
            for (int kk = 0; kk < 2; ++kk) {
                const int fo = kk ? foff1 : foff0;
                bf16x8 wf[TC], xf[TP];
#pragma unroll
                for (int i = 0; i < TC; ++i) wf[i] = *(const bf16x8*)(ws + i * 16 * ROWB + fo);
#pragma unroll
                for (int j = 0; j < TP; ++j) xf[j] = *(const bf16x8*)(xs + j * 16 * ROWB + fo);
#pragma unroll
                for (int i = 0; i < TC; ++i)
#pragma unroll
                    for (int j = 0; j < TP; ++j) {
                        if constexpr (F16) {
                            typedef _Float16 f16x8m __attribute__((ext_vector_type(8)));
                            acc[i][j] = __builtin_amdgcn_mfma_f32_16x16x32_f16(__builtin_bit_cast(f16x8m, wf[i]), __builtin_bit_cast(f16x8m, xf[j]), acc[i][j], 0, 0, 0);
                        } else {
                            acc[i][j] = __builtin_amdgcn_mfma_f32_16x16x32_bf16(wf[i], xf[j], acc[i][j], 0, 0, 0);
                        }
                    }
            }
        }
    }

    const long long ob = (long long)b * a.o_bs;
    const float* resb = a.res ? a.res + (long long)b * a.r_bs : nullptr;
    const f16_t* resh = a.res_f16 ? a.res_f16 + (long long)b * a.r_bs : nullptr;
    const bool wide16 = TC == 4 && (a.ldo % 8) == 0 && (a.o_bs % 8) == 0;
    const bool staged = wide16 && a.out_mode == 0 && (a.out_bf16 || a.out_f16) && c0 + BC <= a.Cout;
    unsigned valid = 0;
    const bool nomask = c0 + BC <= a.Wrows;
#pragma unroll
    for (int j = 0; j < TP; ++j) {
        const int p = p0 + wp * (BP / WP) + j * 16 + frow;
        if (p >= HWo) continue;
        valid |= 1u << j;
        const int cg0 = c0 + wc * (BC / WC) + (TC == 4 ? fq * 16 : fq * 4);
        const float rin = a.row_in ? a.row_in[(long long)b * a.row_bs + p] : 0.f;
        float racc = a.row_mode == 1 ? -__builtin_inff() : 0.f;
        const float alpha2 = a.alpha * 1.44269504f, rin2 = rin * 1.44269504f;
#pragma unroll
        for (int i = 0; i < TC; ++i) {
            const int cg = cg0 + (TC == 4 ? i * 4 : i * 16);
            if (cg >= a.Cout) continue;
            f32x4 v = acc[i][j] * a.alpha;
            if (a.col_scale) v *= *(const f32x4*)(a.col_scale + cg);
            if (a.row_mode) {
                if (a.row_mode == 3) {
                    v *= rin;
                } else if (a.row_mode == 2) {
#pragma unroll
                    for (int r = 0; r < 4; ++r) {
                        const float e = __builtin_amdgcn_exp2f(fmaf(acc[i][j][r], alpha2, -rin2));
                        v[r] = (nomask || cg + r < a.Wrows) ? e : 0.f;
                        racc += v[r];
                    }
                } else {
#pragma unroll
                    for (int r = 0; r < 4; ++r)
                        if (cg + r < a.Wrows) racc = fmaxf(racc, v[r]);
                    continue;
                }
            }
            if (a.bias_mode == 1) {
                const f32x4 bv = *(const f32x4*)(a.bias + cg);
                v += bv;
            } else if (a.bias_mode == 2) {
                const float bv = a.bias[p];
                v += f32x4{bv, bv, bv, bv};
            }
            if (a.out_mode == 1) {
#pragma unroll
                for (int r = 0; r < 4; ++r)
                    if (cg + r < a.cout_keep)
                        a.out_f32[ob + (long long)(cg + r) * HWo + p] = v[r] * a.post_scale + a.post_shift;
                continue;
            }
            const long long o = (long long)p * a.ldo + cg;
            if (resb) {
                const f32x4 rv = *(const f32x4*)(resb + (long long)p * a.ldr + cg);
                v += rv;
            } else if (resh) {
                const f16x4 rh = *(const f16x4*)(resh + (long long)p * a.ldr + cg);
                v += f32x4{(float)rh[0], (float)rh[1], (float)rh[2], (float)rh[3]};
            }
            if (a.out_f32) *(f32x4*)(a.out_f32 + ob + o) = v;
            if (!staged && !(wide16 && cg0 + 16 <= a.Cout)) {
                if (a.out_bf16) {
                    bf16x4 h;
                    h[0] = (bf16_t)v[0]; h[1] = (bf16_t)v[1]; h[2] = (bf16_t)v[2]; h[3] = (bf16_t)v[3];
                    *(bf16x4*)(a.out_bf16 + ob + o) = h;
                }
                if (a.out_f16) {
                    f16x4 h;
                    h[0] = (f16_t)v[0]; h[1] = (f16_t)v[1]; h[2] = (f16_t)v[2]; h[3] = (f16_t)v[3];
                    *(f16x4*)(a.out_f16 + ob + o) = h;
                }
            }
            acc[i][j] = v;
        }
        if (a.row_part) {
            const float o1 = __shfl_xor(racc, 16);
            racc = a.row_mode == 1 ? fmaxf(racc, o1) : racc + o1;
            const float o2 = __shfl_xor(racc, 32);
            racc = a.row_mode == 1 ? fmaxf(racc, o2) : racc + o2;
            const int slots = ctiles * WC;
            if (fq == 0) a.row_part[((long long)b * slots + (c0 / BC) * WC + wc) * a.row_bs + p] = racc;
        }
        if constexpr (TC == 4) {
            if (!staged && wide16 && cg0 + 16 <= a.Cout && a.out_mode == 0) {
                typedef _Float16 f16x8 __attribute__((ext_vector_type(8)));
                const long long o = ob + (long long)p * a.ldo + cg0;
#pragma unroll
                for (int i = 0; i < TC; i += 2) {
                    if (a.out_bf16) {
                        bf16x8 h;
#pragma unroll
                        for (int r = 0; r < 4; ++r) { h[r] = (bf16_t)acc[i][j][r]; h[4 + r] = (bf16_t)acc[i + 1][j][r]; }
                        *(bf16x8*)(a.out_bf16 + o + 4 * i) = h;
                    }
                    if (a.out_f16) {
                        f16x8 h;
#pragma unroll
                        for (int r = 0; r < 4; ++r) { h[r] = (f16_t)acc[i][j][r]; h[4 + r] = (f16_t)acc[i + 1][j][r]; }
                        *(f16x8*)(a.out_f16 + o + 4 * i) = h;
                    }
                }
            }
        }
    }
    if constexpr (TC == 4) {
        if (staged) {
            typedef unsigned u32x4 __attribute__((ext_vector_type(4)));
            typedef _Float16 f16x8 __attribute__((ext_vector_type(8)));
            constexpr int RS = 144, RP = TP * 16 > 64 ? 64 : TP * 16, JP = RP / 16;
            static_assert(8 * RP * RS <= 2 * (BP + BC) * ROWB && (TP % JP) == 0, "staging fits the stage buffers");
            __syncthreads();
            char* R = smem + wave * (RP * RS);
            const int cl = lane & 7, pl = lane >> 3;
            const long long cb = ob + c0 + wc * (BC / WC) + cl * 8;
#pragma unroll
            for (int pass = 0; pass < 2; ++pass) {
                char* outp = pass == 0 ? (char*)a.out_f16 : (char*)a.out_bf16;
                if (!outp) continue;
#pragma unroll
                for (int j0 = 0; j0 < TP; j0 += JP) {
#pragma unroll
                    for (int jj = 0; jj < JP; ++jj)
#pragma unroll
                        for (int i = 0; i < TC; i += 2) {
                            char* d = R + (jj * 16 + frow) * RS + fq * 32 + i * 8;
                            if (pass == 0) {
                                f16x8 h;
#pragma unroll
                                for (int r = 0; r < 4; ++r) { h[r] = (f16_t)acc[i][j0 + jj][r]; h[4 + r] = (f16_t)acc[i + 1][j0 + jj][r]; }
                                *(f16x8*)d = h;
                            } else {
                                bf16x8 h;
#pragma unroll
                                for (int r = 0; r < 4; ++r) { h[r] = (bf16_t)acc[i][j0 + jj][r]; h[4 + r] = (bf16_t)acc[i + 1][j0 + jj][r]; }
                                *(bf16x8*)d = h;
                            }
                        }
                    asm volatile("" ::: "memory");
#pragma unroll
                    for (int k = 0; k < RP / 8; ++k) {
                        const int row = k * 8 + pl;
                        const int p = p0 + wp * (BP / WP) + j0 * 16 + row;
                        const u32x4 v = *(const u32x4*)(R + row * RS + cl * 16);
                        if (p < HWo) *(u32x4*)(outp + (cb + (long long)p * a.ldo) * 2) = v;
                    }
                    asm volatile("" ::: "memory");
                }
            }
        }
    }
    if (a.gn_partial) {
        __syncthreads();
        const int G = a.Cout / a.gn_cpg;
        float* out = a.gn_partial + (((long long)b * ptiles + (p0 / BP)) * G + c0 / a.gn_cpg) * 3;
        if constexpr (TC == 4) vt_gn_epilogue_partials_il<TC, TP>(acc, valid, a.gn_cpg, wp, WP, wc * (BC / WC), BC, (float*)smem, out);
        else vt_gn_epilogue_partials<TC, TP>(acc, valid, a.gn_cpg, wp, WP, wc * (BC / WC), BC, (float*)smem, out);
    }
}

template <int BP, int BC, int WP, int WC, bool OCC2 = false, bool F8 = false, bool F16 = false>
__global__ __launch_bounds__(512, OCC2 ? 4 : 2) void conv_gemm_kernel(const ConvGemmArgs a) {
    extern __shared__ __attribute__((aligned(16))) char smem[];
    conv_gemm_tile<BP, BC, WP, WC, F8, F16>(a, smem, vt_xcd_remap(blockIdx.x, gridDim.x));
}

template <int BP, int BC, int WP, int WC, bool OCC2 = false>
__global__ __launch_bounds__(512, OCC2 ? 4 : 2) void conv_gemm_gated_kernel(const ConvGemmArgs a, int ntiles) {
    extern __shared__ __attribute__((aligned(16))) char smem[];
    if (*a.gate != a.gate_expect) return;
    for (int t = blockIdx.x; t < ntiles; t += gridDim.x) {
        conv_gemm_tile<BP, BC, WP, WC>(a, smem, t);
        __syncthreads();
    }
}

template <int BP, int BC, int WP, int WC, bool OCC2 = false, bool F16 = false>
hipError_t launch_cfg_f8(const ConvGemmArgs& a, hipStream_t s) {
    constexpr int smem = 2 * (BP + BC) * ROWB;
    static std::atomic<unsigned long long> attr_done{0};
    auto kern = conv_gemm_kernel<BP, BC, WP, WC, OCC2, !F16, F16>;
    hipError_t ea = vt_once_per_device(attr_done, [&] { return hipFuncSetAttribute((const void*)kern, hipFuncAttributeMaxDynamicSharedMemorySize, smem); });
    if (ea != hipSuccess) return ea;
    const int HWo = a.Hout * a.Wout;
    const long long nblk = (long long)((HWo + BP - 1) / BP) * ((a.Cout + BC - 1) / BC) * a.batch;
    if (nblk <= 0 || nblk > 0x7fffffffLL) return hipErrorInvalidValue;
    hipLaunchKernelGGL(kern, dim3((unsigned)nblk), dim3(512), smem, s, a);
    return hipGetLastError();
}

template <int BP, int BC, int WP, int WC, bool OCC2 = false>
hipError_t launch_cfg(const ConvGemmArgs& a, hipStream_t s) {
    constexpr int smem = 2 * (BP + BC) * ROWB;
    static_assert(!OCC2 || smem <= 80 * 1024, "two workgroups per CU");
    static std::atomic<unsigned long long> attr_done{0};
    auto kern = conv_gemm_kernel<BP, BC, WP, WC, OCC2>;
    auto gated = conv_gemm_gated_kernel<BP, BC, WP, WC, OCC2>;
    hipError_t ea = vt_once_per_device(attr_done, [&] {
        hipError_t e = hipFuncSetAttribute((const void*)kern, hipFuncAttributeMaxDynamicSharedMemorySize, smem);
        if (e == hipSuccess) e = hipFuncSetAttribute((const void*)gated, hipFuncAttributeMaxDynamicSharedMemorySize, smem);
        return e;
    });
    if (ea != hipSuccess) return ea;
    const int HWo = a.Hout * a.Wout;
    const int ptiles = (HWo + BP - 1) / BP, ctiles = (a.Cout + BC - 1) / BC;
    const long long nblk = (long long)ptiles * ctiles * a.batch;
    if (nblk <= 0 || nblk > 0x7fffffffLL) return hipErrorInvalidValue;
    if (a.gate) hipLaunchKernelGGL(gated, dim3((unsigned)(nblk < 512 ? nblk : 512)), dim3(512), smem, s, a, (int)nblk);
    else hipLaunchKernelGGL(kern, dim3((unsigned)nblk), dim3(512), smem, s, a);
    return hipGetLastError();
}

}

hipError_t vt_launch_conv_gemm(const ConvGemmArgs& a, hipStream_t s) {
    if (!a.X || !a.W || !a.zeros) return hipErrorInvalidValue;
    if (a.ksize != 1 && a.ksize != 3) return hipErrorInvalidValue;
    if (a.Cin <= 0 || a.Cout <= 0 || a.batch <= 0 || a.Wrows <= 0 || a.Wrows > a.Cout) return hipErrorInvalidValue;
    const int ce = a.f8 ? 16 : 8;
    if ((a.ldx % ce) || (a.ldw % ce)) return hipErrorInvalidValue;
    if (a.f8 && (a.gate || a.row_mode || a.x_stream || (a.Cin % 16) || (a.x_bs % 16) || (a.w_bs % 16))) return hipErrorInvalidValue;
    if (a.out_mode == 0 && ((a.ldo % 4) || (a.Cout % 4))) return hipErrorInvalidValue;
    if ((a.res || a.res_f16) && (a.ldr % 4)) return hipErrorInvalidValue;
    if (a.res && a.res_f16) return hipErrorInvalidValue;
    if (a.Cin % 8) return hipErrorInvalidValue;
    if (a.gn_partial) {
        if (a.gn_cpg != 4 && a.gn_cpg != 8 && a.gn_cpg != 16) return hipErrorInvalidValue;
        const int bc = a.Cout <= 32 ? 32 : (a.Cout <= 128 ? 128 : 256);
        if (a.out_mode != 0 || (a.Cout % bc) || a.Cout <= 32) return hipErrorInvalidValue;
    }
    if (a.row_mode < 0 || a.row_mode > 3 || (a.row_mode != 0 && (a.out_mode != 0 || a.gn_partial || a.row_bs < (long long)a.Hout * a.Wout)))
        return hipErrorInvalidValue;
    if ((a.row_mode == 2 || a.row_mode == 3) != (a.row_in != nullptr)) return hipErrorInvalidValue;
    if ((a.row_mode == 1 || a.row_mode == 2) != (a.row_part != nullptr)) return hipErrorInvalidValue;
    if (a.row_mode == 1 && (a.out_f32 || a.out_bf16 || a.out_f16)) return hipErrorInvalidValue;
    if ((long long)a.Hin * a.Win * a.ldx >= (1LL << 31)) return hipErrorInvalidValue;
    if ((long long)a.Wrows * a.ldw >= (1LL << 31)) return hipErrorInvalidValue;
    if (a.f16) {
        if (a.f8 || a.gate || a.row_mode || vt_conv_gemm_config(a) != 0) return hipErrorInvalidValue;
        return launch_cfg_f8<128, 32, 8, 1, false, true>(a, s);
    }
    if (a.f8) {
        switch (vt_conv_gemm_config(a)) {
            case 9: return launch_cfg_f8<192, 128, 4, 2, true>(a, s);
            case 2: return launch_cfg_f8<256, 256, 2, 4>(a, s);
            default: return hipErrorInvalidValue;
        }
    }
    switch (vt_conv_gemm_config(a)) {
        case 0: return launch_cfg<128, 32, 8, 1>(a, s);
        case 1: return launch_cfg<256, 128, 4, 2>(a, s);
        case 9: return launch_cfg<192, 128, 4, 2, true>(a, s);
        default: return launch_cfg<256, 256, 2, 4>(a, s);
    }
}

int vt_conv_gemm_ptiles(int HWo, int Cout) {
    const int bp = Cout <= 32 ? 128 : 192;
    return (HWo + bp - 1) / bp;
}
int vt_conv_gemm_ptiles_of(const ConvGemmArgs& a) {
    const int cfg = vt_conv_gemm_config(a);
    const int bp = cfg == 0 ? 128 : (cfg == 9 ? 192 : 256);
    return (a.Hout * a.Wout + bp - 1) / bp;
}

int vt_conv_gemm_col_slots(const ConvGemmArgs& a) {
    const int cfg = vt_conv_gemm_config(a);
    const int bc = cfg == 0 ? 32 : (cfg == 2 ? 256 : 128), wc = cfg == 0 ? 1 : (cfg == 2 ? 4 : 2);
    return (a.Cout + bc - 1) / bc * wc;
}

int vt_conv_gemm_config(const ConvGemmArgs& a) {
    if (a.Cout <= 32) return 0;
    if (a.Cout == 128 && a.short_tiles && a.ksize == 3 && a.out_mode == 0) return 9;
    if (a.Cout <= 128) return 1;
    if (a.short_tiles && a.ksize == 1 && a.Cin <= 512 && (a.Cout % 128) == 0 && a.out_mode == 0) return 9;
    return 2;
}
const char* vt_conv_gemm_config_name(int cfg) {
    static const char* n[VT_NUM_PROF_SLOTS] = {"conv_gemm_kernel<128,32,8,1>", "conv_gemm_kernel<256,128,4,2>",
                                               "conv_gemm_kernel<256,256,2,4>", "conv3x3_halo_kernel<2,2,0,8,4>",
                                               "conv3x3_halo_kernel<4,2,0,4,4>", "conv3x3_halo_kernel<4,2,0,8,6>",
                                               "conv3x3_halo_kernel<2,4,0,8,6>", "conv3x3_halo_kernel<.,.,1,8,6>",
                                               "conv3x3_halo_kernel<.,.,2,8,6>", "conv_gemm_kernel<192,128,4,2,occ2>", "attn_qk_kernel", "conv3x3_halo_fp8_kernel", "attn_pv_kernel", "conv_gemm_fp8_kernel", "conv3x3_s2_halo_kernel", "attn_qk_fp8_kernel", "attn_pv_fp8_kernel", "conv3x3_s2_halo_fp8_kernel", "proj_fp8_kernel", "conv3x3_halo_fp8_kernel", "attn_qk_kernel<4> (projections)", "conv_out_halo_kernel", "conv3x3_up2_kernel", "gn_apply_kernel"};
    return (cfg >= 0 && cfg < VT_NUM_PROF_SLOTS) ? n[cfg] : "?";
}
```

### vae_tagger_amd/csrc/vt_common.h

```cpp
#pragma once
#include <hip/hip_runtime.h>
#include <stdint.h>

typedef __bf16 bf16_t;
typedef __bf16 bf16x8 __attribute__((ext_vector_type(8)));
typedef __bf16 bf16x4 __attribute__((ext_vector_type(4)));
typedef float f32x4 __attribute__((ext_vector_type(4)));
typedef _Float16 f16_t;
typedef _Float16 f16x4 __attribute__((ext_vector_type(4)));
typedef float f32x16 __attribute__((ext_vector_type(16)));

#include <atomic>
#include <type_traits>
template <typename F>
inline hipError_t vt_once_per_device(std::atomic<unsigned long long>& done, F set) {
    int dev = 0;
    hipError_t e = hipGetDevice(&dev);
    if (e != hipSuccess) return e;
    const unsigned long long bit = 1ull << (dev & 63);
    if (done.load(std::memory_order_acquire) & bit) return hipSuccess;
    e = set();
    if (e != hipSuccess) return e;
    done.fetch_or(bit, std::memory_order_release);
    return hipSuccess;
}

#define VT_GLOBAL_PTR(p) ((const __attribute__((address_space(1))) void*)(p))
#define VT_LDS_PTR(p) ((__attribute__((address_space(3))) void*)(p))

__device__ __forceinline__ float vt_silu(float x) {
    return x * __builtin_amdgcn_rcpf(1.0f + __expf(-x));
}

__device__ __forceinline__ float vt_sigmoid_accurate(float x) { return 1.0f / (1.0f + expf(-x)); }

__device__ __forceinline__ float wave_sum(float v) {
#pragma unroll
    for (int o = 32; o > 0; o >>= 1) v += __shfl_xor(v, o, 64);
    return v;
}
__device__ __forceinline__ float wave_max(float v) {
#pragma unroll
    for (int o = 32; o > 0; o >>= 1) v = fmaxf(v, __shfl_xor(v, o, 64));
    return v;
}

__device__ __forceinline__ double wave_sum_d(double v) {
    for (int d = 32; d > 0; d >>= 1) v += __shfl_down(v, d);
    return v;
}
__device__ __forceinline__ double block_sum_256d(double v, double* red) {
    v = wave_sum_d(v);
    __syncthreads();
    if ((threadIdx.x & 63) == 0) red[threadIdx.x >> 6] = v;
    __syncthreads();
    return ((red[0] + red[1]) + red[2]) + red[3];
}
__device__ __forceinline__ float block_sum_256(float v, float* red) {
    v = wave_sum(v);
    __syncthreads();
    if ((threadIdx.x & 63) == 0) red[threadIdx.x >> 6] = v;
    __syncthreads();
    return (red[0] + red[1]) + (red[2] + red[3]);
}
__device__ __forceinline__ float block_max_256(float v, float* red) {
    v = wave_max(v);
    __syncthreads();
    if ((threadIdx.x & 63) == 0) red[threadIdx.x >> 6] = v;
    __syncthreads();
    return fmaxf(fmaxf(red[0], red[1]), fmaxf(red[2], red[3]));
}

__device__ __forceinline__ int vt_xcd_remap(int id, int n) {
    const int q = n >> 3, r = n & 7, xcd = id & 7, slot = id >> 3;
    const int base = (xcd < r) ? xcd * (q + 1) : r * (q + 1) + (xcd - r) * q;
    return base + slot;
}

__device__ __forceinline__ void vt_chan_merge(float& n, float& mean, float& m2, float nb, float mb, float m2b) {
    if (nb == 0.f) return;
    const float nn = n + nb, d = mb - mean;
    mean += d * (nb / nn);
    m2 += m2b + d * d * (n * nb / nn);
    n = nn;
}

template <int TC, int TP>
__device__ __forceinline__ void vt_gn_epilogue_partials(const f32x4 (&v)[TC][TP], unsigned valid, int cpg, int wp,
                                                        int nwp, int wave_cout0 ,
                                                        int block_couts, float* lds, float* out ) {
    const int lane = threadIdx.x & 63;
    const int fr = lane & 15, fq = lane >> 4;
    const int gpb = block_couts / cpg;
    const float nl = 4.0f * (float)__popc(valid);
#pragma unroll
    for (int i = 0; i < TC; ++i) {
        const float piv = __shfl(v[i][0][0], lane & 48, 64);
        float s = 0.f, ss = 0.f;
#pragma unroll
        for (int j = 0; j < TP; ++j) {
            if ((valid >> j) & 1u) {
#pragma unroll
                for (int r = 0; r < 4; ++r) { const float d = v[i][j][r] - piv; s += d; ss = fmaf(d, d, ss); }
            }
        }
        float n = nl;
#pragma unroll
        for (int o = 1; o < 16; o <<= 1) { s += __shfl_xor(s, o, 64); ss += __shfl_xor(ss, o, 64); n += __shfl_xor(n, o, 64); }
        float mean = 0.f, m2 = 0.f;
        if (n > 0.f) { const float ms = s / n; mean = piv + ms; m2 = fmaxf(ss - s * ms, 0.f); }
        if (cpg >= 8) {
            const float nb = __shfl_xor(n, 16, 64), mb = __shfl_xor(mean, 16, 64), m2b = __shfl_xor(m2, 16, 64);
            if ((fq & 1) == 0) vt_chan_merge(n, mean, m2, nb, mb, m2b);
        }
        if (cpg >= 16) {
            const float nb = __shfl_xor(n, 32, 64), mb = __shfl_xor(mean, 32, 64), m2b = __shfl_xor(m2, 32, 64);
            if (fq == 0) vt_chan_merge(n, mean, m2, nb, mb, m2b);
        }
        const int per = cpg >> 2;
        if (fr == 0 && (fq % per) == 0) {
            const int lg = (wave_cout0 + i * 16 + fq * 4) / cpg;
            float* d = lds + (wp * gpb + lg) * 3;
            d[0] = n; d[1] = mean; d[2] = m2;
        }
    }
    __syncthreads();
    if ((int)threadIdx.x < gpb) {
        float n = 0.f, mean = 0.f, m2 = 0.f;
        for (int w = 0; w < nwp; ++w) {
            const float* d = lds + (w * gpb + threadIdx.x) * 3;
            vt_chan_merge(n, mean, m2, d[0], d[1], d[2]);
        }
        float* o = out + threadIdx.x * 3;
        o[0] = n; o[1] = mean; o[2] = m2;
    }
}

__device__ __forceinline__ float vt_row16_sum(float x) {
    x += __builtin_bit_cast(float, __builtin_amdgcn_update_dpp(0, __builtin_bit_cast(int, x), 0xB1, 0xF, 0xF, true));
    x += __builtin_bit_cast(float, __builtin_amdgcn_update_dpp(0, __builtin_bit_cast(int, x), 0x4E, 0xF, 0xF, true));
    x += __builtin_bit_cast(float, __builtin_amdgcn_update_dpp(0, __builtin_bit_cast(int, x), 0x141, 0xF, 0xF, true));
    x += __builtin_bit_cast(float, __builtin_amdgcn_update_dpp(0, __builtin_bit_cast(int, x), 0x140, 0xF, 0xF, true));
    return x;
}

#if defined(__HIP_DEVICE_COMPILE__)
#define VT_NO_PACKED_F32 __attribute__((target("no-packed-fp32-ops")))
#else
#define VT_NO_PACKED_F32
#endif
#define VT_PIN_PAIR(p2) asm volatile("" : "+v"(p2))
#ifdef GNIL_DUMP
static __device__ float* g_gnil_dump = nullptr;
#endif
template <int TC, int TP>
__device__ __forceinline__ void vt_gn_epilogue_partials_il(const f32x4 (&v)[TC][TP], unsigned valid, int cpg, int wp,
                                                           int nwp, int wave_cout0, int block_couts, float* lds,
                                                           float* out) {
    static_assert(TC == 4, "interleaved map covers 16 couts per lane");
    typedef float f32x2 __attribute__((ext_vector_type(2)));
    const int lane = threadIdx.x & 63;
    const int fr = lane & 15, fq = lane >> 4;
    const int gpb = block_couts / cpg;
    const int tpg = cpg >> 2;
    float n = 0.f;
#pragma unroll
    for (int j = 0; j < TP; ++j) {
        const unsigned long long m = __ballot((valid >> j) & 1u);
        n += (float)__popcll(m & 0xffffull);
    }
    n *= 4.0f * (float)tpg;
    const bool full = __ballot(valid != (1u << TP) - 1u) == 0ull;
    auto partials = [&](auto tpg_tag, auto full_tag) {
        constexpr int TPG = decltype(tpg_tag)::value;
        constexpr bool FULL = decltype(full_tag)::value;
        constexpr int NG = TC / TPG;
        float piv[NG], s[NG], ss[NG];
#pragma unroll
        for (int q = 0; q < NG; ++q) {
#if defined(GNIL_ASM_MODE) && GNIL_ASM_MODE == 3
            const int x0 = __builtin_bit_cast(int, v[q * TPG][0][0]);
            const int r0 = __builtin_amdgcn_readlane(x0, 0), r1 = __builtin_amdgcn_readlane(x0, 16), r2 = __builtin_amdgcn_readlane(x0, 32),
                      r3 = __builtin_amdgcn_readlane(x0, 48);
            piv[q] = __builtin_bit_cast(float, fq == 0 ? r0 : fq == 1 ? r1 : fq == 2 ? r2 : r3);
#else
            piv[q] = __shfl(v[q * TPG][0][0], lane & 48, 64);
#endif
        }
#pragma unroll
        for (int q = 0; q < NG; ++q) {
#ifdef GNIL_ASM_MODE
            f32x2 pr = GNIL_ASM_MODE == 4 ? f32x2{piv[q], 0.f} : f32x2{GNIL_ASM_MODE == 5 ? 1000.f : 0.f, piv[q]};
            const f32x2 a01 = {v[q * TPG][0][0], v[q * TPG][0][1]};
            f32x2 d_first;
#if GNIL_ASM_MODE == 2
            asm volatile("s_waitcnt lgkmcnt(0)\n\ts_nop 7\n\ts_nop 7" : "+v"(pr));
#endif
#if GNIL_ASM_MODE == 4
            asm volatile("v_pk_add_f32 %0, %2, %1 op_sel_hi:[1,0] neg_lo:[0,1] neg_hi:[0,1]" : "=&v"(d_first), "+v"(pr) : "v"(a01));
            piv[q] = pr[0];
#else
            asm volatile("v_pk_add_f32 %0, %2, %1 op_sel:[0,1] neg_lo:[0,1] neg_hi:[0,1]" : "=&v"(d_first), "+v"(pr) : "v"(a01));
            piv[q] = pr[1];
#endif
#endif
            f32x2 p2 = {piv[q], piv[q]};
#ifndef GNIL_OP_SEL_PIVOT
            VT_PIN_PAIR(p2);
#endif
            f32x2 s2 = {0.f, 0.f}, q2 = {0.f, 0.f};
#pragma unroll
            for (int i = q * TPG; i < (q + 1) * TPG; ++i) {
#pragma unroll
                for (int j = 0; j < TP; ++j) {
                    if (FULL || ((valid >> j) & 1u)) {
                        f32x2 d0 = f32x2{v[i][j][0], v[i][j][1]} - p2;
                        const f32x2 d1 = f32x2{v[i][j][2], v[i][j][3]} - p2;
#ifdef GNIL_ASM_MODE
                        if (i == q * TPG && j == 0) d0 = d_first;
#endif
                        s2 += d0; q2 += d0 * d0;
                        s2 += d1; q2 += d1 * d1;
                    }
                }
            }
            s[q] = s2[0] + s2[1]; ss[q] = q2[0] + q2[1];
#ifdef GNIL_DUMP
            if (g_gnil_dump) {
                float* dd = g_gnil_dump + (((long long)blockIdx.x * blockDim.x + threadIdx.x) * 4 + q) * 4;
                dd[0] = s[q]; dd[1] = ss[q]; dd[2] = piv[q]; dd[3] = v[q * TPG][0][0];
            }
#endif
        }
#pragma unroll
        for (int q = 0; q < NG; ++q) { s[q] = vt_row16_sum(s[q]); ss[q] = vt_row16_sum(ss[q]); }
        if (fr == 0) {
            const float rn = n > 0.f ? 1.0f / n : 0.f;
#pragma unroll
            for (int q = 0; q < NG; ++q) {
                const float ms = s[q] * rn;
                const int lg = (wave_cout0 + 16 * fq + 4 * q * TPG) / cpg;
                float* d = lds + (wp * gpb + lg) * 3;
                d[0] = n; d[1] = n > 0.f ? piv[q] + ms : 0.f; d[2] = n > 0.f ? fmaxf(ss[q] - s[q] * ms, 0.f) : 0.f;
            }
        }
    };
    auto partials_f = [&](auto tpg_tag) {
        if (full) partials(tpg_tag, std::true_type{}); else partials(tpg_tag, std::false_type{});
    };
    if (tpg == 1) partials_f(std::integral_constant<int, 1>{});
    else if (tpg == 2) partials_f(std::integral_constant<int, 2>{});
    else partials_f(std::integral_constant<int, 4>{});
    __syncthreads();
    if ((int)threadIdx.x < gpb) {
        float nn = 0.f, mean = 0.f, m2 = 0.f;
        for (int w = 0; w < nwp; ++w) {
            const float* d = lds + (w * gpb + threadIdx.x) * 3;
            vt_chan_merge(nn, mean, m2, d[0], d[1], d[2]);
        }
        float* o = out + threadIdx.x * 3;
        o[0] = nn; o[1] = mean; o[2] = m2;
    }
}

__host__ __device__ inline int vt_halo_step_of_tap(int tap ) { return (tap % 3) * 3 + tap / 3; }

__host__ __device__ inline int vt_s2_step_of_tap(int tap ) { return (int)((0x351786240ULL >> (4 * tap)) & 15); }

__host__ __device__ inline int vt_halo_row_of_cout(int cout_local ) {
    const int r = cout_local & 3, i = (cout_local >> 2) & 3, q = cout_local >> 4;
    return 16 * i + 4 * q + r;
}
```

Before: 217.0.

## Disable packed-f32 codegen, add custom shuffle/barrier helpers and fma_mix residual add

Marks the conv and attention kernels and their lambdas with a no-packed-f32 attribute. Replaces HIP shuffles, ballots and syncthreads with thin builtin wrappers. Adds the f16 residual with v_fma_mix_f32 instead of converting to f32 first, and gives the GroupNorm partials helper a scalar non-paired path, keeping the paired path only for the up2 and gemm callers. The aim is to cut instruction overhead and packed-math codegen issues in the epilogues, at the cost of more inline asm and compiler-specific attributes.

```diff
diff --git a/vae_tagger_amd/csrc/attn_qk.hip b/vae_tagger_amd/csrc/attn_qk.hip
--- a/vae_tagger_amd/csrc/attn_qk.hip
+++ b/vae_tagger_amd/csrc/attn_qk.hip
@@ -14,7 +14,7 @@
 constexpr int KBUF = KT * KROWB;
 
 template <int MODE>
-__global__ __launch_bounds__(512, 2) void attn_qk_kernel(const AttnQkArgs a) {
+__global__ __launch_bounds__(512, 2) VT_NO_PACKED_F32 void attn_qk_kernel(const AttnQkArgs a) {
     extern __shared__ __attribute__((aligned(16))) char smem[];
     if (a.gate && *a.gate != a.gate_expect) return;
     const int lane = threadIdx.x & 63;
@@ -155,7 +155,7 @@
                     }
                 }
                 if (a.gn_partial && kreal) {
-                    const float piv = __shfl(v[0][0], lane & 32, 64);
+                    const float piv = vt_shfl(v[0][0], lane & 32);
                     float s1 = 0.f, s2 = 0.f;
 #pragma unroll
                     for (int j = 0; j < 2; ++j) {
@@ -165,7 +165,7 @@
                         }
                     }
                     s1 = vt_row16_sum(s1); s2 = vt_row16_sum(s2);
-                    s1 += __shfl_xor(s1, 16, 64); s2 += __shfl_xor(s2, 16, 64);
+                    s1 += vt_shfl_xor(s1, 16); s2 += vt_shfl_xor(s2, 16);
                     if (fr == 0 && (fq & 1) == 0) {
                         const float n = (float)nrows * 16.f;
                         const float ms = n > 0.f ? s1 / n : 0.f;
@@ -216,8 +216,8 @@
 #pragma unroll
         for (int j = 0; j < 2; ++j) {
             float v = zero ? 0.f : rv[j];
-            v += __shfl_xor(v, 16);
-            v += __shfl_xor(v, 32);
+            v += vt_shfl_xor(v, 16);
+            v += vt_shfl_xor(v, 32);
             const int row = row0 + j * 16 + fr;
             if (fq == 0 && row < a.S) a.rowout[(long long)seg * a.split_stride + (long long)b * a.row_bs + row] = v;
             rv[j] = 0.f;
@@ -286,9 +286,9 @@
 #pragma unroll
     for (int j = 0; j < 2; ++j) {
         float v = rv[j];
-        const float o1 = __shfl_xor(v, 16);
+        const float o1 = vt_shfl_xor(v, 16);
         v = MODE == 1 ? fmaxf(v, o1) : v + o1;
-        const float o2 = __shfl_xor(v, 32);
+        const float o2 = vt_shfl_xor(v, 32);
         v = MODE == 1 ? fmaxf(v, o2) : v + o2;
         const int row = row0 + j * 16 + fr;
         if (fq == 0 && row < a.S) a.rowout[(long long)b * a.row_bs + row] = MODE == 1 ? v : 1.f / v;
diff --git a/vae_tagger_amd/csrc/conv3x3_halo.hip b/vae_tagger_amd/csrc/conv3x3_halo.hip
--- a/vae_tagger_amd/csrc/conv3x3_halo.hip
+++ b/vae_tagger_amd/csrc/conv3x3_halo.hip
@@ -105,7 +105,7 @@
 }
 
 template <int WP, int WC, int XT, int TPW, int NW, bool F16 = false>
-__global__ __launch_bounds__(64 * WP * WC, TPW == 4 ? 4 : TPW == 16 ? 1 : 2)
+__global__ __launch_bounds__(64 * WP * WC, TPW == 4 ? 4 : TPW == 16 ? 1 : 2) VT_NO_PACKED_F32
 void conv3x3_halo_kernel(const Conv3x3Args a) {
     static_assert(!F16 || XT == 0, "fp16 operands: plain-input tiles only");
     constexpr int NWV = WP * WC;
@@ -141,7 +141,7 @@
 
     STAMP(0);
     const int tiles_x = a.tiles_x, ctiles = a.ctiles, per_img = a.per_img;
-    auto fdiv = [](int n, unsigned long long m, int d) -> int {
+    auto fdiv = [](int n, unsigned long long m, int d) VT_NO_PACKED_F32 -> int {
         return m ? (int)(((unsigned long long)(unsigned)n * m) >> 40) : n / d;
     };
     int logical = vt_xcd_remap(blockIdx.x, gridDim.x);
@@ -180,7 +180,7 @@
     const int wsrc0 = (c0 + wave * 16 + drow) * 32 + dchunk * 8;
     const int wstep = a.Cout * 32;
 
-    auto issue_x_dma = [&](int chunk) {
+    auto issue_x_dma = [&](int chunk) VT_NO_PACKED_F32 {
 #ifdef EXP_NO_DMA
         if (chunk >= 2) return;
 #endif
@@ -202,7 +202,7 @@
         }
     };
     constexpr bool KYMAJOR = XT == 0 && TPW == 4;
-    auto issue_w = [&](int t, int tap_of_t ) {
+    auto issue_w = [&](int t, int tap_of_t ) VT_NO_PACKED_F32 {
 #ifdef EXP_NO_DMA
         if (t >= NW) return;
 #endif
@@ -222,7 +222,7 @@
                 asm volatile("" :: "v"(wt));
 #endif
     };
-    auto load_row = [&](int j, int chunk, f32x4& r0, f32x4& r1) {
+    auto load_row = [&](int j, int chunk, f32x4& r0, f32x4& r1) VT_NO_PACKED_F32 {
         const int xs_j = opaque(xsrc[j]);
         const int off = xs_j >= 0 ? xs_j + chunk * 32 : 0;
         if constexpr (XT == 1) {
@@ -234,7 +234,7 @@
             asm volatile("global_load_dwordx4 %0, %1, off" : "=v"(r0) : "v"(src) : "memory");
         }
     };
-    auto write_row = [&](int j, int chunk, const f32x4& r0, const f32x4& r1) {
+    auto write_row = [&](int j, int chunk, const f32x4& r0, const f32x4& r1) VT_NO_PACKED_F32 {
         const float* sp = ssl + (chunk * 32 + opaque(dchunk) * 8) * 2;
         char* dst = xbase + (chunk & 1) * XBUF + (j * NLD + wave) * 1024 + opaque(lane) * 16;
         const bool pad = xsrc[j] < 0;
@@ -281,7 +281,7 @@
 #pragma unroll
     for (int k = 0; k < 8; ++k)
         xsel[k] = (wp * TPW * HWID + fr) * HB + ((fq ^ ((((k + fr) >> 2) & 1) << 1)) << 4);
-    auto xaddr = [&](int k) -> int { return xsel[k]; };
+    auto xaddr = [&](int k) VT_NO_PACKED_F32 -> int { return xsel[k]; };
     f32x4 acc[TC][TP];
 #pragma unroll
     for (int i = 0; i < TC; ++i) {
@@ -292,7 +292,7 @@
     if constexpr (XT != 0) {
         const float* ssg = a.scale_shift + (long long)b * a.Cin * 2;
         for (int i = threadIdx.x; i < a.Cin * 2; i += NT) ssl[i] = ssg[i];
-        __syncthreads();
+        vt_syncthreads();
 #pragma unroll
         for (int j = 0; j < NXW; ++j) {
             f32x4 r0 = {0.f, 0.f, 0.f, 0.f}, r1 = {0.f, 0.f, 0.f, 0.f};
@@ -328,7 +328,7 @@
     STAMP(2);
     STAMP_CLK(11);
 
-    auto do_chunk = [&](int chunk, auto last_tag) {
+    auto do_chunk = [&](int chunk, auto last_tag) VT_NO_PACKED_F32 {
         constexpr bool LAST = decltype(last_tag)::value;
         const char* xs = xbase + (chunk & 1) * XBUF;
         const int tbase = chunk * 9;
@@ -390,7 +390,7 @@
                 const int dx_n = (dx + 1) % 3;
                 const char* xs_n = (dx == 2) ? xbase + ((chunk + 1) & 1) * XBUF : xs;
                 const char* ws_n = wbase + ((t + 1) % NW) * WBUF + opaque(wfoff);
-                auto refill = [&](int r) {
+                auto refill = [&](int r) VT_NO_PACKED_F32 {
 #ifndef EXP_NO_FRAG_READS
                     const int rel = r * HWID + dx_n;
                     xr[r] = *(const bf16x8*)(xs_n + xaddr(rel & 7) + rel * HB);
@@ -429,7 +429,7 @@
 
             constexpr bool STAGE = !LAST && XT != 0;
             const int r = tap - DLY;
-            auto stage_row = [&]() {
+            auto stage_row = [&]() VT_NO_PACKED_F32 {
                 int n = DLY * wpw;
                 for (int q = r + 1; q < tap; ++q) if (q < NXW) n += LX;
                 if constexpr (XT == 1) wait_vmcnt_tied(n, rq[r % DLY][0], rq[r % DLY][1]);
@@ -537,7 +537,7 @@
     char* const rbuf = smem + wave * (RPCS * 1024);
     if (RES_DMA && a.res_f16) {
         asm volatile("s_waitcnt lgkmcnt(0)" ::: "memory");
-        __syncthreads();
+        vt_syncthreads();
 #pragma unroll 4
         for (int pc = 0; pc < RPCS; ++pc) {
             const int pp = pc * 8 + (lane >> 3);
@@ -567,11 +567,16 @@
             const int pp = j * 16 + fr;
 #pragma unroll
             for (int i = 0; i < TC; i += 2) {
-                typedef _Float16 f16x8 __attribute__((ext_vector_type(8)));
-                const f16x8 rh = RES_DMA ? *(const f16x8*)(rbuf + pp * 128 + (((2 * fq + (i >> 1)) ^ (pp & 7)) << 4))
-                                         : *(const f16x8*)(a.res_f16 + o + 4 * i);
-#pragma unroll
-                for (int r = 0; r < 4; ++r) { acc[i][j][r] += (float)rh[r]; acc[i + 1][j][r] += (float)rh[4 + r]; }
+                typedef unsigned u32x4 __attribute__((ext_vector_type(4)));
+                const u32x4 rh = RES_DMA ? *(const u32x4*)(rbuf + pp * 128 + (((2 * fq + (i >> 1)) ^ (pp & 7)) << 4))
+                                         : *(const u32x4*)(a.res_f16 + o + 4 * i);
+#pragma unroll
+                for (int r = 0; r < 4; r += 2) {
+                    acc[i][j][r] = vt_add_f16_half<0>(acc[i][j][r], rh[r >> 1]);
+                    acc[i][j][r + 1] = vt_add_f16_half<1>(acc[i][j][r + 1], rh[r >> 1]);
+                    acc[i + 1][j][r] = vt_add_f16_half<0>(acc[i + 1][j][r], rh[2 + (r >> 1)]);
+                    acc[i + 1][j][r + 1] = vt_add_f16_half<1>(acc[i + 1][j][r + 1], rh[2 + (r >> 1)]);
+                }
             }
         }
         if (a.out_f16) {
@@ -609,7 +614,7 @@
     }
     STAMP(4);
     if (a.gn_partial) {
-        __syncthreads();
+        vt_syncthreads();
         STAMP(10);
         const int G = a.Cout / a.gn_cpg;
         float* out = a.gn_partial + (((long long)b * a.ptiles + tile) * G + c0 / a.gn_cpg) * 3;
diff --git a/vae_tagger_amd/csrc/conv3x3_s2_halo.hip b/vae_tagger_amd/csrc/conv3x3_s2_halo.hip
--- a/vae_tagger_amd/csrc/conv3x3_s2_halo.hip
+++ b/vae_tagger_amd/csrc/conv3x3_s2_halo.hip
@@ -20,20 +20,20 @@
 constexpr int SMEM = NXB * XSTRIDE + NW * WBUF;
 static_assert(2 * SMEM <= 160 * 1024, "two workgroups per CU");
 
-__host__ __device__ constexpr int pl_py(int pl) { return pl >> 1; }
-__host__ __device__ constexpr int pl_px(int pl) { return pl & 1; }
-__host__ __device__ constexpr int pl_pitch(int pl) { return pl_px(pl) ? 16 : 17; }
-__host__ __device__ constexpr int pl_hrows(int pl) { return pl_py(pl) ? 16 : 17; }
-__host__ __device__ constexpr int pl_rows(int pl) { return pl_pitch(pl) * pl_hrows(pl); }
-__host__ __device__ constexpr int pl_pieces(int pl) { return pl_rows(pl) / 16; }
-__host__ __device__ constexpr int nx_pl(int pl) { return pl == 3 ? 4 : 5; }
-__host__ __device__ constexpr int st_plane(int p) { return p < 4 ? 0 : p < 6 ? 1 : p < 8 ? 2 : 3; }
-__host__ __device__ constexpr int st_dx(int p) { return (p == 2 || p == 3 || p == 7) ? 1 : 0; }
-__host__ __device__ constexpr int st_dy(int p) { return (p == 1 || p == 3 || p == 5) ? 1 : 0; }
-__host__ __device__ constexpr bool st_two(int p) { return p < 6; }
-__host__ __device__ constexpr int ng_plane(int p) { return p < 2 ? 0 : p < 4 ? 1 : p < 7 ? 2 : p < 8 ? 3 : 0; }
-__host__ __device__ constexpr int ng_dx(int p) { return (p < 2 || p == 6) ? 1 : 0; }
-__host__ __device__ constexpr int ng_rows(int p) { return (p < 4 || p == 8) ? 9 : 8; }
+__host__ __device__ constexpr __attribute__((always_inline)) int pl_py(int pl) { return pl >> 1; }
+__host__ __device__ constexpr __attribute__((always_inline)) int pl_px(int pl) { return pl & 1; }
+__host__ __device__ constexpr __attribute__((always_inline)) int pl_pitch(int pl) { return pl_px(pl) ? 16 : 17; }
+__host__ __device__ constexpr __attribute__((always_inline)) int pl_hrows(int pl) { return pl_py(pl) ? 16 : 17; }
+__host__ __device__ constexpr __attribute__((always_inline)) int pl_rows(int pl) { return pl_pitch(pl) * pl_hrows(pl); }
+__host__ __device__ constexpr __attribute__((always_inline)) int pl_pieces(int pl) { return pl_rows(pl) / 16; }
+__host__ __device__ constexpr __attribute__((always_inline)) int nx_pl(int pl) { return pl == 3 ? 4 : 5; }
+__host__ __device__ constexpr __attribute__((always_inline)) int st_plane(int p) { return p < 4 ? 0 : p < 6 ? 1 : p < 8 ? 2 : 3; }
+__host__ __device__ constexpr __attribute__((always_inline)) int st_dx(int p) { return (p == 2 || p == 3 || p == 7) ? 1 : 0; }
+__host__ __device__ constexpr __attribute__((always_inline)) int st_dy(int p) { return (p == 1 || p == 3 || p == 5) ? 1 : 0; }
+__host__ __device__ constexpr __attribute__((always_inline)) bool st_two(int p) { return p < 6; }
+__host__ __device__ constexpr __attribute__((always_inline)) int ng_plane(int p) { return p < 2 ? 0 : p < 4 ? 1 : p < 7 ? 2 : p < 8 ? 3 : 0; }
+__host__ __device__ constexpr __attribute__((always_inline)) int ng_dx(int p) { return (p < 2 || p == 6) ? 1 : 0; }
+__host__ __device__ constexpr __attribute__((always_inline)) int ng_rows(int p) { return (p < 4 || p == 8) ? 9 : 8; }
 
 __device__ __forceinline__ void wait_vmcnt(int n) {
     switch (n) {
@@ -53,7 +53,7 @@
 }
 
 template <bool F16>
-__global__ __launch_bounds__(NT, 2) void conv3x3_s2_halo_kernel(const Conv3x3S2Args a) {
+__global__ __launch_bounds__(NT, 2) VT_NO_PACKED_F32 void conv3x3_s2_halo_kernel(const Conv3x3S2Args a) {
     extern __shared__ __attribute__((aligned(16))) char smem[];
     char* const xbase = smem;
     char* const wbase = smem + NXB * XSTRIDE;
@@ -62,7 +62,7 @@
     const int wp = wave / WC, wc = wave % WC;
     const int fr = lane & 15, fq = lane >> 4;
 
-    auto fdiv = [](int n, unsigned long long m, int d) -> int {
+    auto fdiv = [](int n, unsigned long long m, int d) VT_NO_PACKED_F32 -> int {
         return m ? (int)(((unsigned long long)(unsigned)n * m) >> 40) : n / d;
     };
     int logical = vt_xcd_remap(blockIdx.x, gridDim.x);
@@ -83,7 +83,7 @@
     const int wsrc0 = (c0 + wave * 16 + drow) * 32 + dchunk * 8;
     const int wstep = a.Cout * 32;
 
-    auto issue_x = [&](auto pl_tag, int chunk, int slot) {
+    auto issue_x = [&](auto pl_tag, int chunk, int slot) VT_NO_PACKED_F32 {
         constexpr int PL = decltype(pl_tag)::value;
         constexpr int PITCH = pl_pitch(PL), PY = pl_py(PL), PX = pl_px(PL), NP = pl_pieces(PL), NXP = nx_pl(PL);
         constexpr int NPT = PL == 0 ? NP + 1 : NP;
@@ -101,7 +101,7 @@
             __builtin_amdgcn_global_load_lds(VT_GLOBAL_PTR(src), VT_LDS_PTR(dst + row0 * HB), 16, 0, 0);
         }
     };
-    auto issue_w = [&](int t) {
+    auto issue_w = [&](int t) VT_NO_PACKED_F32 {
         char* dst = wbase + (t % NW) * WBUF;
         const bf16_t* wt = a.Wp + (long long)t * wstep + opaque(wsrc0);
 #pragma unroll
@@ -120,11 +120,11 @@
 #pragma unroll
     for (int k = 0; k < 8; ++k) xsel[k] = fr * HB + ((fq ^ ((((k + fr) >> 2) & 1) << 1)) << 4);
     const int wpoff17 = wp * TP * 17 * HB, wpoff16 = wp * TP * 16 * HB;
-    auto xfrag = [&](const char* buf , int pitch , int r, int dx) -> bf16x8 {
+    auto xfrag = [&](const char* buf , int pitch , int r, int dx) VT_NO_PACKED_F32 -> bf16x8 {
         const int rel = r * pitch + dx;
         return *(const bf16x8*)(buf + xsel[rel & 7] + rel * HB);
     };
-    auto xfrag_after = [&](const char* buf, int pitch, int r, int dx, const f32x4& after) -> bf16x8 {
+    auto xfrag_after = [&](const char* buf, int pitch, int r, int dx, const f32x4& after) VT_NO_PACKED_F32 -> bf16x8 {
         const int rel = r * pitch + dx;
         int off = xsel[rel & 7];
         asm volatile("" : "+v"(off) : "v"(after));
@@ -151,9 +151,9 @@
     }
 
     int cm = 0;
-    auto slot_of = [&](int cmod, int pl) -> int { const int s = cmod + pl; return s >= 3 ? (s >= 6 ? s - 6 : s - 3) : s; };
-
-    auto do_chunk = [&](int chunk, auto last_tag) {
+    auto slot_of = [&](int cmod, int pl) VT_NO_PACKED_F32 -> int { const int s = cmod + pl; return s >= 3 ? (s >= 6 ? s - 6 : s - 3) : s; };
+
+    auto do_chunk = [&](int chunk, auto last_tag) VT_NO_PACKED_F32 {
         constexpr bool LAST = decltype(last_tag)::value;
         const int tbase = chunk * 9;
         const int cmn = cm == 2 ? 0 : cm + 1;
@@ -181,7 +181,7 @@
             const char* xs_n = xbase + opaque_s(slot_of(next_chunk ? cmn : cm, npl) * XSTRIDE + (npitch == 17 ? wpoff17 : wpoff16));
             const char* ws_n = wbase + ((t + 1) % NW) * WBUF + opaque(wfoff);
             (void)pl;
-            auto refill = [&](int r, const f32x4& after) {
+            auto refill = [&](int r, const f32x4& after) VT_NO_PACKED_F32 {
                 if (has_next && r < nrows) xr[r] = xfrag_after(xs_n, npitch, r, ndx, after);
             };
             __builtin_amdgcn_s_setprio(1);
@@ -281,7 +281,7 @@
     }
     if (a.gn_partial) {
         asm volatile("s_waitcnt lgkmcnt(0)" ::: "memory");
-        __syncthreads();
+        vt_syncthreads();
         const int G = a.Cout / a.gn_cpg;
         float* out = a.gn_partial + (((long long)b * a.ptiles + tile) * G + c0 / a.gn_cpg) * 3;
         vt_gn_epilogue_partials_il<TC, TP>(acc, valid, a.gn_cpg, wp, WP, wc * 64, BC, (float*)smem, out);
diff --git a/vae_tagger_amd/csrc/conv3x3_up2.hip b/vae_tagger_amd/csrc/conv3x3_up2.hip
--- a/vae_tagger_amd/csrc/conv3x3_up2.hip
+++ b/vae_tagger_amd/csrc/conv3x3_up2.hip
@@ -167,7 +167,7 @@
         __syncthreads();
         const int G = a.Cout / a.gn_cpg;
         float* out = a.gn_partial + (((long long)b * a.ptiles + tile) * G + c0 / a.gn_cpg) * 3;
-        vt_gn_epilogue_partials_il<TC, 8>(acc, valid, a.gn_cpg, wave, NWV, 0, BC, (float*)smem, out);
+        vt_gn_epilogue_partials_il<TC, 8, true>(acc, valid, a.gn_cpg, wave, NWV, 0, BC, (float*)smem, out);
     }
 }
 
diff --git a/vae_tagger_amd/csrc/conv_gemm.hip b/vae_tagger_amd/csrc/conv_gemm.hip
--- a/vae_tagger_amd/csrc/conv_gemm.hip
+++ b/vae_tagger_amd/csrc/conv_gemm.hip
@@ -325,7 +325,7 @@
         __syncthreads();
         const int G = a.Cout / a.gn_cpg;
         float* out = a.gn_partial + (((long long)b * ptiles + (p0 / BP)) * G + c0 / a.gn_cpg) * 3;
-        if constexpr (TC == 4) vt_gn_epilogue_partials_il<TC, TP>(acc, valid, a.gn_cpg, wp, WP, wc * (BC / WC), BC, (float*)smem, out);
+        if constexpr (TC == 4) vt_gn_epilogue_partials_il<TC, TP, true>(acc, valid, a.gn_cpg, wp, WP, wc * (BC / WC), BC, (float*)smem, out);
         else vt_gn_epilogue_partials<TC, TP>(acc, valid, a.gn_cpg, wp, WP, wc * (BC / WC), BC, (float*)smem, out);
     }
 }
diff --git a/vae_tagger_amd/csrc/vt_common.h b/vae_tagger_amd/csrc/vt_common.h
--- a/vae_tagger_amd/csrc/vt_common.h
+++ b/vae_tagger_amd/csrc/vt_common.h
@@ -150,15 +150,43 @@
 #define VT_NO_PACKED_F32
 #endif
 #define VT_PIN_PAIR(p2) asm volatile("" : "+v"(p2))
+__device__ __forceinline__ void vt_syncthreads() {
+    __builtin_amdgcn_fence(__ATOMIC_RELEASE, "workgroup");
+    __builtin_amdgcn_s_barrier();
+    __builtin_amdgcn_fence(__ATOMIC_ACQUIRE, "workgroup");
+}
+__device__ __forceinline__ float vt_shfl(float v, int src_lane) {
+    const int self = __builtin_amdgcn_mbcnt_hi(-1, __builtin_amdgcn_mbcnt_lo(-1, 0));
+    const int index = (src_lane & 63) + (self & ~63);
+    return __builtin_bit_cast(float, __builtin_amdgcn_ds_bpermute(index << 2, __builtin_bit_cast(int, v)));
+}
+__device__ __forceinline__ float vt_shfl_xor(float v, int lane_mask) {
+    const int self = __builtin_amdgcn_mbcnt_hi(-1, __builtin_amdgcn_mbcnt_lo(-1, 0));
+    int index = self ^ lane_mask;
+    index = index >= ((self + 64) & ~63) ? self : index;
+    return __builtin_bit_cast(float, __builtin_amdgcn_ds_bpermute(index << 2, __builtin_bit_cast(int, v)));
+}
+__device__ __forceinline__ unsigned long long vt_ballot(bool p) { return __builtin_amdgcn_ballot_w64(p); }
+template <int H>
+__device__ __forceinline__ float vt_add_f16_half(float acc, unsigned h2) {
+    static_assert(H == 0 || H == 1, "low or high half");
+#if defined(__HIP_DEVICE_COMPILE__) && !defined(VT_NO_FMA_MIX)
+    if (H == 0) asm("v_fma_mix_f32 %0, %1, 1.0, %0 op_sel:[0,0,0] op_sel_hi:[1,0,0]" : "+v"(acc) : "v"(h2));
+    else asm("v_fma_mix_f32 %0, %1, 1.0, %0 op_sel:[1,0,0] op_sel_hi:[1,0,0]" : "+v"(acc) : "v"(h2));
+    return acc;
+#else
+    typedef _Float16 f16x2 __attribute__((ext_vector_type(2)));
+    return acc + (float)__builtin_bit_cast(f16x2, h2)[H];
+#endif
+}
 #ifdef GNIL_DUMP
 static __device__ float* g_gnil_dump = nullptr;
 #endif
-template <int TC, int TP>
+template <int TC, int TP, bool PAIRED = false>
 __device__ __forceinline__ void vt_gn_epilogue_partials_il(const f32x4 (&v)[TC][TP], unsigned valid, int cpg, int wp,
                                                            int nwp, int wave_cout0, int block_couts, float* lds,
                                                            float* out) {
     static_assert(TC == 4, "interleaved map covers 16 couts per lane");
-    typedef float f32x2 __attribute__((ext_vector_type(2)));
     const int lane = threadIdx.x & 63;
     const int fr = lane & 15, fq = lane >> 4;
     const int gpb = block_couts / cpg;
@@ -166,65 +194,56 @@
     float n = 0.f;
 #pragma unroll
     for (int j = 0; j < TP; ++j) {
-        const unsigned long long m = __ballot((valid >> j) & 1u);
-        n += (float)__popcll(m & 0xffffull);
+        const unsigned long long m = vt_ballot((valid >> j) & 1u);
+        n += (float)__builtin_popcountll(m & 0xffffull);
     }
     n *= 4.0f * (float)tpg;
-    const bool full = __ballot(valid != (1u << TP) - 1u) == 0ull;
-    auto partials = [&](auto tpg_tag, auto full_tag) {
+    const bool full = vt_ballot(valid != (1u << TP) - 1u) == 0ull;
+    auto partials = [&](auto tpg_tag, auto full_tag) __attribute__((always_inline)) {
         constexpr int TPG = decltype(tpg_tag)::value;
         constexpr bool FULL = decltype(full_tag)::value;
         constexpr int NG = TC / TPG;
         float piv[NG], s[NG], ss[NG];
 #pragma unroll
+        for (int q = 0; q < NG; ++q) piv[q] = vt_shfl(v[q * TPG][0][0], lane & 48);
+#pragma unroll
         for (int q = 0; q < NG; ++q) {
-#if defined(GNIL_ASM_MODE) && GNIL_ASM_MODE == 3
-            const int x0 = __builtin_bit_cast(int, v[q * TPG][0][0]);
-            const int r0 = __builtin_amdgcn_readlane(x0, 0), r1 = __builtin_amdgcn_readlane(x0, 16), r2 = __builtin_amdgcn_readlane(x0, 32),
-                      r3 = __builtin_amdgcn_readlane(x0, 48);
-            piv[q] = __builtin_bit_cast(float, fq == 0 ? r0 : fq == 1 ? r1 : fq == 2 ? r2 : r3);
-#else
-            piv[q] = __shfl(v[q * TPG][0][0], lane & 48, 64);
-#endif
-        }
-#pragma unroll
-        for (int q = 0; q < NG; ++q) {
-#ifdef GNIL_ASM_MODE
-            f32x2 pr = GNIL_ASM_MODE == 4 ? f32x2{piv[q], 0.f} : f32x2{GNIL_ASM_MODE == 5 ? 1000.f : 0.f, piv[q]};
-            const f32x2 a01 = {v[q * TPG][0][0], v[q * TPG][0][1]};
-            f32x2 d_first;
-#if GNIL_ASM_MODE == 2
-            asm volatile("s_waitcnt lgkmcnt(0)\n\ts_nop 7\n\ts_nop 7" : "+v"(pr));
-#endif
-#if GNIL_ASM_MODE == 4
-            asm volatile("v_pk_add_f32 %0, %2, %1 op_sel_hi:[1,0] neg_lo:[0,1] neg_hi:[0,1]" : "=&v"(d_first), "+v"(pr) : "v"(a01));
-            piv[q] = pr[0];
-#else
-            asm volatile("v_pk_add_f32 %0, %2, %1 op_sel:[0,1] neg_lo:[0,1] neg_hi:[0,1]" : "=&v"(d_first), "+v"(pr) : "v"(a01));
-            piv[q] = pr[1];
-#endif
-#endif
-            f32x2 p2 = {piv[q], piv[q]};
-#ifndef GNIL_OP_SEL_PIVOT
-            VT_PIN_PAIR(p2);
-#endif
-            f32x2 s2 = {0.f, 0.f}, q2 = {0.f, 0.f};
-#pragma unroll
-            for (int i = q * TPG; i < (q + 1) * TPG; ++i) {
-#pragma unroll
-                for (int j = 0; j < TP; ++j) {
-                    if (FULL || ((valid >> j) & 1u)) {
-                        f32x2 d0 = f32x2{v[i][j][0], v[i][j][1]} - p2;
-                        const f32x2 d1 = f32x2{v[i][j][2], v[i][j][3]} - p2;
-#ifdef GNIL_ASM_MODE
-                        if (i == q * TPG && j == 0) d0 = d_first;
-#endif
-                        s2 += d0; q2 += d0 * d0;
-                        s2 += d1; q2 += d1 * d1;
+            if constexpr (PAIRED) {
+                typedef float f32x2 __attribute__((ext_vector_type(2)));
+                f32x2 p2 = {piv[q], piv[q]};
+                VT_PIN_PAIR(p2);
+                f32x2 s2 = {0.f, 0.f}, q2 = {0.f, 0.f};
+#pragma unroll
+                for (int i = q * TPG; i < (q + 1) * TPG; ++i) {
+#pragma unroll
+                    for (int j = 0; j < TP; ++j) {
+                        if (FULL || ((valid >> j) & 1u)) {
+                            const f32x2 d0 = f32x2{v[i][j][0], v[i][j][1]} - p2;
+                            const f32x2 d1 = f32x2{v[i][j][2], v[i][j][3]} - p2;
+                            s2 += d0; q2 += d0 * d0;
+                            s2 += d1; q2 += d1 * d1;
+                        }
                     }
                 }
-            }
-            s[q] = s2[0] + s2[1]; ss[q] = q2[0] + q2[1];
+                s[q] = s2[0] + s2[1]; ss[q] = q2[0] + q2[1];
+            } else {
+                const float p = piv[q];
+                float s0 = 0.f, s1 = 0.f, q0 = 0.f, q1 = 0.f;
+#pragma unroll
+                for (int i = q * TPG; i < (q + 1) * TPG; ++i) {
+#pragma unroll
+                    for (int j = 0; j < TP; ++j) {
+                        if (FULL || ((valid >> j) & 1u)) {
+                            const float d0 = v[i][j][0] - p, d1 = v[i][j][1] - p, d2 = v[i][j][2] - p, d3 = v[i][j][3] - p;
+                            s0 += d0; q0 = __builtin_fmaf(d0, d0, q0);
+                            s1 += d1; q1 = __builtin_fmaf(d1, d1, q1);
+                            s0 += d2; q0 = __builtin_fmaf(d2, d2, q0);
+                            s1 += d3; q1 = __builtin_fmaf(d3, d3, q1);
+                        }
+                    }
+                }
+                s[q] = s0 + s1; ss[q] = q0 + q1;
+            }
 #ifdef GNIL_DUMP
             if (g_gnil_dump) {
                 float* dd = g_gnil_dump + (((long long)blockIdx.x * blockDim.x + threadIdx.x) * 4 + q) * 4;
@@ -245,13 +264,13 @@
             }
         }
     };
-    auto partials_f = [&](auto tpg_tag) {
+    auto partials_f = [&](auto tpg_tag) __attribute__((always_inline)) {
         if (full) partials(tpg_tag, std::true_type{}); else partials(tpg_tag, std::false_type{});
     };
     if (tpg == 1) partials_f(std::integral_constant<int, 1>{});
     else if (tpg == 2) partials_f(std::integral_constant<int, 2>{});
     else partials_f(std::integral_constant<int, 4>{});
-    __syncthreads();
+    vt_syncthreads();
     if ((int)threadIdx.x < gpb) {
         float nn = 0.f, mean = 0.f, m2 = 0.f;
         for (int w = 0; w < nwp; ++w) {
@@ -263,11 +282,11 @@
     }
 }
 
-__host__ __device__ inline int vt_halo_step_of_tap(int tap ) { return (tap % 3) * 3 + tap / 3; }
-
-__host__ __device__ inline int vt_s2_step_of_tap(int tap ) { return (int)((0x351786240ULL >> (4 * tap)) & 15); }
-
-__host__ __device__ inline int vt_halo_row_of_cout(int cout_local ) {
+__host__ __device__ inline __attribute__((always_inline)) int vt_halo_step_of_tap(int tap ) { return (tap % 3) * 3 + tap / 3; }
+
+__host__ __device__ inline __attribute__((always_inline)) int vt_s2_step_of_tap(int tap ) { return (int)((0x351786240ULL >> (4 * tap)) & 15); }
+
+__host__ __device__ inline __attribute__((always_inline)) int vt_halo_row_of_cout(int cout_local ) {
     const int r = cout_local & 3, i = (cout_local >> 2) & 3, q = cout_local >> 4;
     return 16 * i + 4 * q + r;
 }
```

Result: no change. 217.7, median of 6 (+0.3%).
